# DecaYale/SYN3R

Hardware: AMD Instinct MI355X
Metric: llff_3view_train_loop_iters_per_sec (higher is better)
Workload: dtype f32 raster / f16 UNet (f32 accumulate); 1 GPU; LLFF fern-like 3-view block: 50 raster fwd+bwd iters (l1 loss) (200000 Gaussians, 1920x1080, SH3) + 1 SVD (step,pass): CFG UNet fwd [2,14,8,72,128] f16 + fused Euler step; frames=14, parallelism=scene-parallel x1

## Files before the change

### include/syn3r_hip.h

```cpp
#ifndef SYN3R_HIP_H
#define SYN3R_HIP_H

#include <stddef.h>
#include <stdint.h>

#ifdef __cplusplus
extern "C" {
#endif

#define SYN3R_OK 0
#define SYN3R_E_INVALID (-1)
#define SYN3R_E_WORKSPACE (-2)
#define SYN3R_E_HIP (-3)

#define SYN3R_F32 0
#define SYN3R_F16 1

const char* syn3r_last_error(void);
int syn3r_version(void);
const char* syn3r_arch(void);

int syn3r_trace_enable(int on);
void* syn3r_trace_session(void);
int syn3r_trace_attach(void* session);
// ... 114 lines not shown
                              const float* projmatrix, const float* campos, float tanfovx, float tanfovy, int H, int W,
                              const float* bg, const int* radii, void* geom, size_t geom_bytes,
                              const unsigned* point_list, void* image, size_t image_bytes, const float* dL_dcolor,
                              const float* dL_ddepth, const float* dL_dalpha, float* dL_dmeans3D, float* dL_dscales,
                              float* dL_drotations, float* dL_dopacities, float* dL_dshs, float* dL_dmeans2D,
                              float* dL_dconfidence, void* workspace, size_t workspace_bytes, int raw, int flags,
                              const float* filter3d, void* stream);
int syn3r_raster_backward_abs(int N, int sh_degree, int sh_coeffs, long long P, const float* means3D,
                              const float* scales, const float* rotations, const float* opacities, const float* shs,
                              const float* confidence, float scale_modifier, const float* viewmatrix,
                              const float* projmatrix, const float* campos, float tanfovx, float tanfovy, int H, int W,
                              const float* bg, const int* radii, void* geom, size_t geom_bytes,
                              const unsigned* point_list, void* image, size_t image_bytes, const float* dL_dcolor,
                              const float* dL_ddepth, const float* dL_dalpha, float* dL_dmeans3D, float* dL_dscales,
                              float* dL_drotations, float* dL_dopacities, float* dL_dshs, float* dL_dmeans2D,
                              float* dL_dconfidence, void* workspace, size_t workspace_bytes, int raw, int flags,
                              const float* filter3d, float* dL_dmeans2D_abs, void* stream);
size_t syn3r_raster_backward_cam_workspace_bytes(int N);
int syn3r_raster_backward_cam(int N, int sh_degree, int sh_coeffs, long long P, const float* means3D,
                              const float* scales, const float* rotations, const float* opacities, const float* shs,
                              const float* confidence, float scale_modifier, const float* viewmatrix,
                              const float* projmatrix, const float* campos, float tanfovx, float tanfovy, int H, int W,
                              const float* bg, const int* radii, void* geom, size_t geom_bytes,
                              const unsigned* point_list, void* image, size_t image_bytes, const float* dL_dcolor,
                              const float* dL_ddepth, const float* dL_dalpha, float* dL_dmeans3D, float* dL_dscales,
                              float* dL_drotations, float* dL_dopacities, float* dL_dshs, float* dL_dmeans2D,
                              float* dL_dconfidence, void* workspace, size_t workspace_bytes, int raw, int flags,
                              const float* filter3d, float* dL_dmeans2D_abs, float* dL_dcamera, int accumulate,
                              void* stream);

size_t syn3r_sort_pairs_workspace_bytes(long long n);
int syn3r_sort_pairs(unsigned long long* keys, unsigned* vals, unsigned long long* keys_tmp, unsigned* vals_tmp,
                     long long n, int nbits, void* workspace, size_t workspace_bytes, int* result_in_tmp,
                     void* stream);


int syn3r_gemm_f16(const void* A, long long lda, const void* W, void* out, long long ldc, const void* bias,
                   const void* rowvec, long long ldrv, int rows_per_vec, int rv_group_rows, const void* residual, long long ldr,
                   const void* aux, long long ldaux, float s_acc, float s_res, float s_aux, int M, int N, int K,
                   void* gn_partials, size_t gn_partials_bytes, int* gn_written, void* stream);

int syn3r_gemm_2src_supported(int M, int N, int K1, int K2, long long lda1, long long lda2);
int syn3r_gemm_2src_f16(const void* A1, long long lda1, int K1, const void* A2, long long lda2, int K2, const void* W,
                        void* out, long long ldc, const void* bias, int M, int N, void* gn_partials, size_t gn_partials_bytes,
                        int* gn_written, void* stream);

int syn3r_gemm_set_tile(int bm);

int syn3r_gemm_set_splitk_workspace(void* workspace, size_t bytes);

int syn3r_gemm_geglu_f16(const void* A, long long lda, const void* Wpacked, const void* bias_packed, void* out,
                         long long ldc, int M, int D, int K, void* stream);

size_t syn3r_feedforward_workspace_bytes(int M, int D);
int syn3r_feedforward_f16(const void* x, long long ldx, const void* w1_packed, const void* b1_packed, int D,
                          const void* w2, const void* b2, void* out, long long ldc, const void* residual,
                          long long ldr, const void* aux, long long ldaux, float s_acc, float s_res, float s_aux,
                          int M, int C_in, int C_out, void* workspace, size_t workspace_bytes, void* stream);

int syn3r_feedforward_p64_supported(int M, int D, int C_in);
int syn3r_feedforward_p64_f16(const void* x, long long ldx, const void* w1_packed64, const void* b1_packed64, int D,
                              const void* w2, const void* b2, void* out, long long ldc, const void* residual,
                              long long ldr, const void* aux, long long ldaux, float s_acc, float s_res, float s_aux,
                              int M, int C_in, int C_out, void* workspace, size_t workspace_bytes, void* stream);

int syn3r_feedforward_fused_f16(const void* x, long long ldx, const void* w1_chunked, const void* b1_chunked, int D,
                                const void* w2, const void* b2, void* out, long long ldc, const void* residual,
                                long long ldr, const void* aux, long long ldaux, float s_acc, float s_res, float s_aux,
                                int M, int C, void* stream);

int syn3r_feedforward_fused_ln_f16(const void* x, long long ldx, const void* ln_gamma, const void* ln_beta, float ln_eps,
                                   const void* w1_chunked, const void* b1_chunked, int D, const void* w2, const void* b2,
                                   void* out, long long ldc, const void* residual, long long ldr, const void* aux,
                                   long long ldaux, float s_acc, float s_res, float s_aux, int M, int C, void* stream);

int syn3r_feedforward_fused_addln_f16(const void* x, long long ldx, const void* addvec, int rows_per_vec, const void* ln_gamma,
                                      const void* ln_beta, float ln_eps, const void* w1_chunked, const void* b1_chunked, int D,
                                      const void* w2, const void* b2, void* out, long long ldc, const void* aux, long long ldaux,
                                      float s_acc, float s_res, float s_aux, int M, int C, void* stream);

int syn3r_layernorm_linear320_f16(const void* x, long long ldx, const void* ln_gamma, const void* ln_beta, float ln_eps,
                                  const void* W, void* out, long long ldc, int M, int N, int C, void* stream);

int syn3r_conv2d3x3_f16(const void* X, const void* W, void* out, long long ldc, const void* bias,
                        const void* rowvec, long long ldrv, int rows_per_vec, const void* residual, long long ldr,
                        float s_acc, float s_res, int NB, int Hi, int Wi, int Cin, int Cout, int stride, int upsample,
                        int pad_lo, void* gn_partials, size_t gn_partials_bytes, int* gn_written, void* stream);

int syn3r_pack_upsample4_f16(const void* w, void* w4, int Cout, int Cin);
int syn3r_conv2d3x3_up4_f16(const void* X, const void* w4, void* out, const void* bias, const void* residual, int NB, int Hi, int Wi,
                            int Cin, int Cout, void* gn_partials, size_t gn_partials_bytes, int* gn_written, void* stream);

int syn3r_tconv3_f16(const void* X, const void* W, void* out, long long ldc, const void* bias, const void* rowvec,
                     long long ldrv, int rows_per_vec, const void* residual, long long ldr, float s_acc, float s_res,
                     int B, int F, int HW, int Cin, int Cout, void* gn_partials, size_t gn_partials_bytes, int* gn_written,
                     void* stream);

int syn3r_attention_f16(const void* q, const void* k, const void* v, long long ld, void* out, long long ldo,
                        int nseq, int S, int heads, void* stream);

int syn3r_attention_temporal_f16(const void* q, const void* k, const void* v, long long ld, void* out,
                                 long long ldo, int B, int F, int HW, int heads, void* stream);

size_t syn3r_groupnorm_workspace_bytes(int samples, int rows);
int syn3r_groupnorm_f16(const void* x, void* y, int samples, int rows, int C, const void* gamma, const void* beta,
                        float eps, int silu, void* workspace, size_t workspace_bytes, void* stream);
int syn3r_groupnorm_2src_f16(const void* x1, int C1, const void* x2, int C2, void* y, int samples, int rows,
                             const void* gamma, const void* beta, float eps, int silu, void* workspace,
                             size_t workspace_bytes, void* stream);
size_t syn3r_gn_partials_bytes(int M, int N);
int syn3r_groupnorm_pre_f16(const void* x1, int C1, const void* part1, const void* x2, int C2, const void* part2, void* y,
                            int samples, int rows, const void* gamma, const void* beta, float eps, int silu,
                            void* workspace, size_t workspace_bytes, void* stream);

int syn3r_layernorm_f16(const void* x, void* y, void* xsum, const void* addvec, int rows_per_vec, long long M,
                        int C, const void* gamma, const void* beta, float eps, void* stream);

int syn3r_geglu_f16(const void* x, void* y, long long M, int D, void* stream);

int syn3r_softmax_rows_f16(const void* x, void* y, long long M, int N, long long ld, float scale, void* stream);

int syn3r_time_conv_out(const void* x, long long ldx, const float* w, const float* bias, float* out, int B, int F,
                        long long HW, void* stream);


size_t syn3r_l1_loss_workspace_bytes(long long n);
int syn3r_l1_loss(const float* image, const float* target, long long n, float weight, float* loss, void* ws,
                  size_t ws_bytes, void* stream);
int syn3r_l1_loss_backward(const float* image, const float* target, long long n, float weight,
                           const float* grad_loss, float* grad_image, void* stream);

int syn3r_image_mse(const float* image, const float* target, long long n, float* mse, void* ws, size_t ws_bytes,
                    void* stream);

size_t syn3r_photo_loss_workspace_bytes(int C, int H, int W);
int syn3r_photo_loss(const float* image, const float* target, int C, int H, int W, float lambda_dssim, float weight,
                     float* loss3, void* ws, size_t ws_bytes, void* stream);
int syn3r_photo_loss_backward(const float* image, const float* target, int C, int H, int W, float lambda_dssim,
                              float weight, const float* grad_loss, const void* ws, float* grad_image, void* stream);
int syn3r_photo_loss_step(const float* image, const float* target, int C, int H, int W, float lambda_dssim, float weight,
                          const float* grad_loss, float* loss3, float* grad_image, void* ws, size_t ws_bytes, void* stream);

size_t syn3r_photo_loss_map_workspace_bytes(int C, int H, int W);
int syn3r_photo_loss_map(const float* image, const float* target, const float* map, int C, int H, int W, float lambda_dssim,
                         float weight, float* loss4, void* ws, size_t ws_bytes, void* stream);
int syn3r_photo_loss_map_backward(const float* image, const float* target, const float* map, int C, int H, int W,
                                  float lambda_dssim, float weight, const float* grad_loss, const void* ws, float* grad_image,
                                  void* stream);
int syn3r_photo_loss_map_step(const float* image, const float* target, const float* map, int C, int H, int W, float lambda_dssim,
                              float weight, const float* grad_loss, float* loss4, float* grad_image, void* ws, size_t ws_bytes,
                              void* stream);
int syn3r_l1_loss_map(const float* image, const float* target, const float* map, long long n, long long plane, float weight,
                      float* loss, void* ws, size_t ws_bytes, void* stream);
int syn3r_l1_loss_map_backward(const float* image, const float* target, const float* map, long long n, long long plane,
                               float weight, const float* grad_loss, float* grad_image, void* stream);

#define SYN3R_DCORR_MIN 0
#define SYN3R_DCORR_A 1
#define SYN3R_DCORR_B 2
size_t syn3r_depth_corr_loss_workspace_bytes(long long n);
int syn3r_depth_corr_loss(const float* depth, const float* prior, long long n, float weight, float offset, int mode, float* parts,
                          void* ws, size_t ws_bytes, void* stream);
int syn3r_depth_corr_loss_backward(const float* depth, const float* prior, long long n, float weight, float offset, int mode,
                                   const float* grad_loss, const void* ws, size_t ws_bytes, float* grad_depth, void* stream);
int syn3r_depth_corr_loss_step(const float* depth, const float* prior, long long n, float weight, float offset, int mode,
                               const float* grad_loss, float* parts, float* grad_depth, void* ws, size_t ws_bytes, void* stream);
// ... 127 lines not shown
```

### syn3r_amd/_lib.py

```python
from __future__ import annotations

import ctypes as C
from pathlib import Path

import torch

_LIB_PATH = Path(__file__).resolve().parent / "lib" / "libsyn3r_hip.so"
_lib = None

c_f = C.c_float
c_i = C.c_int
c_p = C.c_void_p
c_sz = C.c_size_t
c_ll = C.c_longlong
c_d = C.c_double

F32, F16 = 0, 1
RASTER_ANTIALIAS = 1

FILTER3D_VARIANCE, FILTER3D_NEAR, FILTER3D_MARGIN = 0.2, 0.2, 0.15

_SCENE = [c_p, c_p, c_p, c_p, c_p, c_p, c_f, c_p, c_p, c_p, c_f, c_f, c_i, c_i]
_RASTER_PREPROCESS = [c_i, c_i, c_i] + _SCENE + [c_p, c_p, c_sz, C.POINTER(c_ll)]
_RASTER_BACKWARD = ([c_i, c_i, c_i, c_ll] + _SCENE + [c_p, c_p, c_p, c_sz, c_p, c_p, c_sz]
                    + [c_p] * 10 + [c_p, c_sz])
_STREAM, _EX, _F3D, _ABS = [c_p], [c_i, c_i, c_p], [c_i, c_i, c_p, c_p], [c_i, c_i, c_p, c_p, c_p]
_CAM = [c_i, c_i, c_p, c_p, c_p, c_i, c_p]
CAMERA_GRAD = 35

SIGNATURES = {
    "syn3r_last_error": (C.c_char_p, []),
    "syn3r_version": (c_i, []),
    "syn3r_arch": (C.c_char_p, []),
    "syn3r_trace_enable": (c_i, [c_i]),
    "syn3r_trace_filter": (c_i, [C.c_char_p]),
    "syn3r_trace_report": (c_i, [C.c_char_p, c_sz]),
    "syn3r_trace_session": (c_p, []),
    "syn3r_trace_attach": (c_i, [c_p]),
    "syn3r_inverse_warp_workspace_bytes": (c_sz, [c_i]),
    "syn3r_inverse_warp": (c_i, [c_p, c_p, c_p, c_p, c_p, c_p, c_p, c_f, c_i, c_i, c_i,
                                 c_p, c_p, c_p, c_p, c_p, c_p, c_p, c_p, c_p, c_p, c_p, c_p, c_sz, c_p]),
    "syn3r_reproj_error": (c_i, [c_p, c_p, c_p, c_p, c_p, c_p, c_p, c_i, c_i, c_p, c_p]),
    "syn3r_warp_post": (c_i, [c_p, c_p, c_p, c_i, c_i, c_i, c_i, c_i, c_p, c_p, c_p, c_p, c_p, c_p, c_p]),
    "syn3r_fuse_uncertainty": (c_i, [c_p, c_p, c_p, c_i, c_i, c_i, c_i, c_i, c_p, c_p, c_p, c_p]),
    "syn3r_forward_warp_workspace_bytes": (c_sz, [c_i, c_i]),
    "syn3r_forward_warp": (c_i, [c_p, c_p, c_p, c_p, c_p, c_p, c_i, c_i, c_p, c_p, c_p, c_p, c_sz, c_p]),
    "syn3r_step_workspace_bytes": (c_sz, [c_i, c_i, c_i, c_i]),
    "syn3r_step_interp": (c_i, [c_p, c_i, c_p, c_i, c_p, c_p, c_p, c_f, c_f, c_f, c_f, c_f, c_f, c_i,
                                c_p, c_p, c_p, c_i, c_i, c_i, c_i, c_p, c_sz, c_p]),
    "syn3r_step_replace": (c_i, [c_p, c_i, c_p, c_i, c_p, c_p, c_p, c_f, c_f, c_f, c_f,
                                 c_p, c_p, c_i, c_i, c_i, c_i, c_p, c_sz, c_p]),
    "syn3r_raster_geom_bytes": (c_sz, [c_i]),
    "syn3r_raster_image_bytes": (c_sz, [c_i, c_i]),
    "syn3r_raster_binning_bytes": (c_sz, [c_ll]),
    "syn3r_raster_preprocess": (c_i, _RASTER_PREPROCESS + _STREAM),
    "syn3r_raster_preprocess_raw": (c_i, _RASTER_PREPROCESS + _STREAM),
    "syn3r_raster_preprocess_ex": (c_i, _RASTER_PREPROCESS + _EX),
    "syn3r_raster_preprocess_f3d": (c_i, _RASTER_PREPROCESS + _F3D),
    "syn3r_raster_render": (c_i, [c_i, c_i, c_i, c_p, c_p, c_p, c_sz, c_p, c_sz, c_p, c_sz, c_ll, c_p, c_p, c_p,
                                  C.POINTER(c_p), c_p]),
    "syn3r_raster_backward_workspace_bytes": (c_sz, [c_i]),
    "syn3r_raster_backward": (c_i, _RASTER_BACKWARD + _STREAM),
    "syn3r_raster_backward_raw": (c_i, _RASTER_BACKWARD + _STREAM),
    "syn3r_raster_backward_ex": (c_i, _RASTER_BACKWARD + _EX),
    "syn3r_raster_backward_f3d": (c_i, _RASTER_BACKWARD + _F3D),
    "syn3r_raster_backward_abs": (c_i, _RASTER_BACKWARD + _ABS),
    "syn3r_raster_backward_cam_workspace_bytes": (c_sz, [c_i]),
    "syn3r_raster_backward_cam": (c_i, _RASTER_BACKWARD + _CAM),
    "syn3r_filter3d_workspace_bytes": (c_sz, [c_i]),
    "syn3r_filter3d_compute": (c_i, [c_p, c_i, c_p, c_i, c_f, c_f, c_f, c_p, c_p, c_sz, c_p]),
    "syn3r_sort_pairs_workspace_bytes": (c_sz, [c_ll]),
    "syn3r_sort_pairs": (c_i, [c_p, c_p, c_p, c_p, c_ll, c_i, c_p, c_sz, C.POINTER(c_i), c_p]),
    "syn3r_gaussian_activate": (c_i, [c_i, c_p, c_p, c_p, c_p, c_p, c_p, c_p]),
    "syn3r_gaussian_activate_backward": (c_i, [c_i, c_p, c_p, c_p, c_p, c_p, c_p, c_p, c_p, c_p, c_p, c_p]),
    "syn3r_densification_stats": (c_i, [c_i, c_p, c_p, c_p, c_p, c_p, c_p]),
    "syn3r_densification_stats_abs": (c_i, [c_i, c_p, c_p, c_p, c_p, c_p, c_p, c_p, c_p]),
    "syn3r_gemm_f16": (c_i, [c_p, c_ll, c_p, c_p, c_ll, c_p, c_p, c_ll, c_i, c_i, c_p, c_ll, c_p, c_ll, c_f, c_f, c_f,
                             c_i, c_i, c_i, c_p, c_sz, C.POINTER(c_i), c_p]),
    "syn3r_gemm_set_tile": (c_i, [c_i]),
    "syn3r_gemm_geglu_f16": (c_i, [c_p, c_ll, c_p, c_p, c_p, c_ll, c_i, c_i, c_i, c_p]),
    "syn3r_feedforward_workspace_bytes": (c_sz, [c_i, c_i]),
    "syn3r_feedforward_f16": (c_i, [c_p, c_ll, c_p, c_p, c_i, c_p, c_p, c_p, c_ll, c_p, c_ll, c_p, c_ll, c_f, c_f, c_f,
                                    c_i, c_i, c_i, c_p, c_sz, c_p]),
    "syn3r_feedforward_p64_f16": (c_i, [c_p, c_ll, c_p, c_p, c_i, c_p, c_p, c_p, c_ll, c_p, c_ll, c_p, c_ll, c_f, c_f, c_f,
                                    c_i, c_i, c_i, c_p, c_sz, c_p]),
    "syn3r_feedforward_p64_supported": (c_i, [c_i, c_i, c_i]),
    "syn3r_feedforward_fused_f16": (c_i, [c_p, c_ll, c_p, c_p, c_i, c_p, c_p, c_p, c_ll, c_p, c_ll, c_p, c_ll, c_f, c_f, c_f,
                                          c_i, c_i, c_p]),
    "syn3r_feedforward_fused_ln_f16": (c_i, [c_p, c_ll, c_p, c_p, c_f, c_p, c_p, c_i, c_p, c_p, c_p, c_ll, c_p, c_ll, c_p, c_ll,
                                             c_f, c_f, c_f, c_i, c_i, c_p]),
    "syn3r_feedforward_fused_addln_f16": (c_i, [c_p, c_ll, c_p, c_i, c_p, c_p, c_f, c_p, c_p, c_i, c_p, c_p, c_p, c_ll, c_p, c_ll,
                                                c_f, c_f, c_f, c_i, c_i, c_p]),
    "syn3r_layernorm_linear320_f16": (c_i, [c_p, c_ll, c_p, c_p, c_f, c_p, c_p, c_ll, c_i, c_i, c_i, c_p]),
    "syn3r_conv2d3x3_f16": (c_i, [c_p, c_p, c_p, c_ll, c_p, c_p, c_ll, c_i, c_p, c_ll, c_f, c_f,
                                  c_i, c_i, c_i, c_i, c_i, c_i, c_i, c_i, c_p, c_sz, C.POINTER(c_i), c_p]),
    "syn3r_pack_upsample4_f16": (c_i, [c_p, c_p, c_i, c_i]),
    "syn3r_conv2d3x3_up4_f16": (c_i, [c_p, c_p, c_p, c_p, c_p, c_i, c_i, c_i, c_i, c_i, c_p, c_sz, C.POINTER(c_i), c_p]),
    "syn3r_tconv3_f16": (c_i, [c_p, c_p, c_p, c_ll, c_p, c_p, c_ll, c_i, c_p, c_ll, c_f, c_f,
                               c_i, c_i, c_i, c_i, c_i, c_p, c_sz, C.POINTER(c_i), c_p]),
    "syn3r_attention_f16": (c_i, [c_p, c_p, c_p, c_ll, c_p, c_ll, c_i, c_i, c_i, c_p]),
    "syn3r_attention_temporal_f16": (c_i, [c_p, c_p, c_p, c_ll, c_p, c_ll, c_i, c_i, c_i, c_i, c_p]),
    "syn3r_groupnorm_workspace_bytes": (c_sz, [c_i, c_i]),
    "syn3r_groupnorm_f16": (c_i, [c_p, c_p, c_i, c_i, c_i, c_p, c_p, c_f, c_i, c_p, c_sz, c_p]),
    "syn3r_groupnorm_2src_f16": (c_i, [c_p, c_i, c_p, c_i, c_p, c_i, c_i, c_p, c_p, c_f, c_i, c_p, c_sz, c_p]),
    "syn3r_groupnorm_pre_f16": (c_i, [c_p, c_i, c_p, c_p, c_i, c_p, c_p, c_i, c_i, c_p, c_p, c_f, c_i, c_p, c_sz, c_p]),
    "syn3r_gn_partials_bytes": (c_sz, [c_i, c_i]),
    "syn3r_gemm_2src_supported": (c_i, [c_i, c_i, c_i, c_i, c_ll, c_ll]),
    "syn3r_gemm_2src_f16": (c_i, [c_p, c_ll, c_i, c_p, c_ll, c_i, c_p, c_p, c_ll, c_p, c_i, c_i, c_p, c_sz, C.POINTER(c_i), c_p]),
    "syn3r_layernorm_f16": (c_i, [c_p, c_p, c_p, c_p, c_i, c_ll, c_i, c_p, c_p, c_f, c_p]),
    "syn3r_geglu_f16": (c_i, [c_p, c_p, c_ll, c_i, c_p]),
    "syn3r_softmax_rows_f16": (c_i, [c_p, c_p, c_ll, c_i, c_ll, c_f, c_p]),
    "syn3r_time_conv_out": (c_i, [c_p, c_ll, c_p, c_p, c_p, c_i, c_i, c_ll, c_p]),
    "syn3r_l1_loss_workspace_bytes": (c_sz, [c_ll]),
    "syn3r_l1_loss": (c_i, [c_p, c_p, c_ll, c_f, c_p, c_p, c_sz, c_p]),
    "syn3r_l1_loss_backward": (c_i, [c_p, c_p, c_ll, c_f, c_p, c_p, c_p]),
    "syn3r_image_mse": (c_i, [c_p, c_p, c_ll, c_p, c_p, c_sz, c_p]),
    "syn3r_photo_loss_workspace_bytes": (c_sz, [c_i, c_i, c_i]),
    "syn3r_photo_loss": (c_i, [c_p, c_p, c_i, c_i, c_i, c_f, c_f, c_p, c_p, c_sz, c_p]),
    "syn3r_photo_loss_backward": (c_i, [c_p, c_p, c_i, c_i, c_i, c_f, c_f, c_p, c_p, c_p, c_p]),
    "syn3r_photo_loss_step": (c_i, [c_p, c_p, c_i, c_i, c_i, c_f, c_f, c_p, c_p, c_p, c_p, c_sz, c_p]),
    "syn3r_photo_loss_map_workspace_bytes": (c_sz, [c_i, c_i, c_i]),
    "syn3r_photo_loss_map": (c_i, [c_p, c_p, c_p, c_i, c_i, c_i, c_f, c_f, c_p, c_p, c_sz, c_p]),
    "syn3r_photo_loss_map_backward": (c_i, [c_p, c_p, c_p, c_i, c_i, c_i, c_f, c_f, c_p, c_p, c_p, c_p]),
    "syn3r_photo_loss_map_step": (c_i, [c_p, c_p, c_p, c_i, c_i, c_i, c_f, c_f, c_p, c_p, c_p, c_p, c_sz, c_p]),
    "syn3r_l1_loss_map": (c_i, [c_p, c_p, c_p, c_ll, c_ll, c_f, c_p, c_p, c_sz, c_p]),
    "syn3r_l1_loss_map_backward": (c_i, [c_p, c_p, c_p, c_ll, c_ll, c_f, c_p, c_p, c_p]),
    "syn3r_depth_corr_loss_workspace_bytes": (c_sz, [c_ll]),
    "syn3r_depth_corr_loss": (c_i, [c_p, c_p, c_ll, c_f, c_f, c_i, c_p, c_p, c_sz, c_p]),
    "syn3r_depth_corr_loss_backward": (c_i, [c_p, c_p, c_ll, c_f, c_f, c_i, c_p, c_p, c_sz, c_p, c_p]),
    "syn3r_depth_corr_loss_step": (c_i, [c_p, c_p, c_ll, c_f, c_f, c_i, c_p, c_p, c_p, c_p, c_sz, c_p]),
    "syn3r_depth_corr_local_workspace_bytes": (c_sz, [c_i, c_i, c_i, c_i, c_i]),
    "syn3r_depth_corr_local_loss": (c_i, [c_p, c_p, c_i, c_i, c_i, c_i, c_i, c_f, c_f, c_i, c_p, c_p, c_sz, c_p]),
    "syn3r_depth_corr_local_loss_backward": (c_i, [c_p, c_p, c_i, c_i, c_i, c_i, c_i, c_f, c_f, c_i, c_p, c_p, c_sz, c_p, c_i, c_p]),
    "syn3r_depth_corr_local_loss_step": (c_i, [c_p, c_p, c_i, c_i, c_i, c_i, c_i, c_f, c_f, c_i, c_p, c_p, c_p, c_i, c_p, c_sz, c_p]),
    "syn3r_exposure_apply": (c_i, [c_p, c_p, c_i, c_i, c_p, c_p]),
    "syn3r_depth_edge_weights": (c_i, [c_p, c_i, c_i, c_f, c_p, c_p]),
    "syn3r_depth_smooth_workspace_bytes": (c_sz, [c_i, c_i]),
    "syn3r_depth_smooth_loss": (c_i, [c_p, c_p, c_i, c_i, c_f, c_p, c_p, c_sz, c_p]),
    "syn3r_depth_smooth_loss_backward": (c_i, [c_p, c_p, c_i, c_i, c_f, c_p, c_p, c_sz, c_p, c_i, c_p]),
    "syn3r_depth_smooth_loss_step": (c_i, [c_p, c_p, c_i, c_i, c_f, c_p, c_p, c_p, c_i, c_p, c_sz, c_p]),
    "syn3r_photo_reproj_workspace_bytes": (c_sz, [c_i, c_i, c_i]),
    "syn3r_photo_reproj_loss": (c_i, [c_p, c_p, c_p, c_p, c_p, c_p, c_i, c_i, c_i, c_f, c_f, c_p, c_p, c_sz, c_p]),
    "syn3r_photo_reproj_loss_backward": (c_i, [c_p, c_p, c_i, c_i, c_i, c_f, c_f, c_p, c_p, c_sz, c_p, c_i, c_p, c_i, c_p]),
    "syn3r_photo_reproj_loss_step": (c_i, [c_p, c_p, c_p, c_p, c_p, c_p, c_i, c_i, c_i, c_f, c_f, c_p, c_p, c_p, c_i, c_p, c_i, c_p, c_sz,
                                           c_p]),
    "syn3r_exposure_backward_workspace_bytes": (c_sz, [c_i, c_i]),
    "syn3r_exposure_backward": (c_i, [c_p, c_p, c_p, c_i, c_i, c_p, c_p, c_i, c_p, c_sz, c_p]),
    "syn3r_mcmc_noise": (c_i, [c_p, c_p, c_p, c_p, c_i, c_f, c_ll, c_i, c_p]),
    "syn3r_mcmc_reg_step_workspace_bytes": (c_sz, [c_i]),
    "syn3r_mcmc_reg_step": (c_i, [c_p, c_p, c_i, c_f, c_f, c_p, c_p, c_p, c_p, c_sz, c_p]),
    "syn3r_mcmc_weights": (c_i, [c_p, c_i, c_f, c_p, c_p]),
    "syn3r_mcmc_sample_workspace_bytes": (c_sz, [c_i]),
    "syn3r_mcmc_sample": (c_i, [c_p, c_i, c_i, c_ll, c_i, c_p, c_p, c_p, c_sz, c_p]),
    "syn3r_mcmc_relocate": (c_i, [c_i, c_p, c_p, c_p, c_p, c_i, c_p, c_p, c_p, c_p, c_f, c_p]),
    "syn3r_adam_step": (c_i, [c_p, c_p, c_p, c_p, c_ll, c_f, c_f, c_f, c_f, c_i, c_p]),
    "syn3r_adam_step_multi": (c_i, [c_i, c_p, c_p, c_p, c_p, c_p, c_p, c_f, c_f, c_p, c_p, c_p]),
    "syn3r_adam_step_multi_rows": (c_i, [c_i, c_p, c_p, c_p, c_p, c_p, c_p, c_p, c_p, c_p, c_f, c_f, c_p, c_p, c_p]),
    "syn3r_knn3_workspace_bytes": (c_sz, [c_i]),
    "syn3r_knn3_mean_dist2": (c_i, [c_p, c_i, c_p, c_p, c_sz, c_p]),
    "syn3r_knn3_graph_workspace_bytes": (c_sz, [c_i]),
    "syn3r_knn3_graph": (c_i, [c_p, c_i, c_p, c_p, c_p, c_sz, c_p]),
    "syn3r_gaussian_unpool_workspace_bytes": (c_sz, [c_i]),
    "syn3r_gaussian_unpool_count": (c_i, [c_p, c_p, c_i, c_f, c_f, c_p, c_p, c_sz, c_p]),
    "syn3r_gaussian_unpool_emit": (c_i, [c_p, c_p, c_p, c_p, c_p, c_i, c_i, c_i, c_p, c_p, c_p, c_p, c_p, c_p, c_sz, c_p]),
    "syn3r_conv2d3x3_act_f16": (c_i, [c_p, c_p, c_p, c_p, c_i, c_p, c_i, c_i, c_i, c_i, c_i, c_p]),
    "syn3r_lpips_image_f16": (c_i, [c_p, c_i, c_i, c_p, c_p]),
    "syn3r_lpips_image_bwd": (c_i, [c_p, c_i, c_i, c_f, c_p, c_p]),
    "syn3r_maxpool2_f16": (c_i, [c_p, c_i, c_i, c_i, c_p, c_p]),
    "syn3r_maxpool2_bwd_f16": (c_i, [c_p, c_p, c_i, c_i, c_i, c_p, c_p]),
    "syn3r_lpips_layer_workspace_bytes": (c_sz, [c_ll, c_i]),
    "syn3r_lpips_layer_f16": (c_i, [c_p, c_p, c_p, c_ll, c_i, c_i, c_p, c_p, c_sz, c_p]),
    "syn3r_lpips_layer_bwd_f16": (c_i, [c_p, c_p, c_p, c_ll, c_i, c_f, c_i, c_p, c_p]),
    "syn3r_conv2d3x3_split_f16": (c_i, [c_p, c_p, c_p, c_ll, c_p, c_i, c_i, c_p, c_ll, c_i, c_i, c_i, c_i, c_i, c_p]),
    "syn3r_lpips_image_split_f16": (c_i, [c_p, c_i, c_i, c_p, c_p]),
    "syn3r_maxpool2_split_f16": (c_i, [c_p, c_i, c_i, c_i, c_p, c_p]),
    "syn3r_maxpool2_bwd_split_f16": (c_i, [c_p, c_p, c_i, c_i, c_i, c_p, c_p]),
# ... 144 lines not shown
```

### syn3r_amd/csrc/attn.hip

```cpp
#include "common.h"
#include <type_traits>

using namespace syn3r;

namespace {

typedef _Float16 half8 __attribute__((ext_vector_type(8)));
typedef _Float16 half4 __attribute__((ext_vector_type(4)));
typedef float float16v __attribute__((ext_vector_type(16)));
typedef float float2v __attribute__((ext_vector_type(2)));
typedef __fp16 fp16x4 __attribute__((__vector_size__(4 * sizeof(__fp16))));

__device__ __forceinline__ int v_off(int key, int d) { return key * 64 + ((((d >> 3) ^ (((key >> 1) & 1) << 2)) << 3) | (d & 7)); }
__device__ __forceinline__ int k_off(int key, int chunk) { return key * 64 + ((chunk ^ ((key >> 1) & 7)) << 3); }

__device__ __forceinline__ half8 v_frag_tr(const __half* vs, int r0, int d0, int lane) {
    const int i = lane & 15, q = i >> 2, pc = i & 3;
    const int c = d0 + ((lane >> 4) & 1) * 16 + 4 * pc;
    typedef __attribute__((address_space(3))) fp16x4 lds4;
    fp16x4 a = __builtin_amdgcn_ds_read_tr16_b64_v4f16((lds4*)(vs + v_off(r0 + q, c)));
    fp16x4 b = __builtin_amdgcn_ds_read_tr16_b64_v4f16((lds4*)(vs + v_off(r0 + 8 + q, c)));
    half8 r;
#pragma unroll
    for (int e = 0; e < 4; ++e) { r[e] = (_Float16)a[e]; r[4 + e] = (_Float16)b[e]; }
    return r;
}

constexpr float kNegBig = -1.0e30f;
constexpr float kLog2e = 1.4426950408889634f;
constexpr float kLazy = 8.0f;

__device__ __forceinline__ half8 pack8(const float16v& p, int s) {
    half8 r;
#pragma unroll
    for (int j = 0; j < 8; ++j) r[j] = (_Float16)p[8 * s + j];
    return r;
}

struct AttnParams {
    const __half* q; const __half* k; const __half* v;
    long long ld;
    __half* o; long long ldo;
    int S;
    int nseq;
    int heads;
    int F, HW;
};

constexpr int BQ = 128, BKV = 64, ATHREADS = 256;

typedef float float4v __attribute__((ext_vector_type(4)));
typedef __attribute__((address_space(3))) void lds_void_t;
typedef __attribute__((address_space(1))) const void gbl_void_t;

#ifndef ATTN_WAVES
#define ATTN_WAVES 3
#endif
__device__ __forceinline__ float max3(float a, float b, float c) {
    float d;
    asm("v_max3_f32 %0, %1, %2, %3" : "=v"(d) : "v"(a), "v"(b), "v"(c));
    return d;
}
__device__ __forceinline__ int v16_off(int key, int d) { return key * 64 + ((((d >> 4) ^ ((key >> 1) & 3)) << 4) | (d & 15)); }

__device__ __forceinline__ half8 v16_frag_tr(const __half* vs, int r0, int d0, int lane) {
    const int i = lane & 15, q = i >> 2, pc = i & 3;
    const int c = d0 + 4 * pc;
    typedef __attribute__((address_space(3))) fp16x4 lds4;
    fp16x4 a = __builtin_amdgcn_ds_read_tr16_b64_v4f16((lds4*)(vs + v16_off(r0 + q, c)));
    fp16x4 b = __builtin_amdgcn_ds_read_tr16_b64_v4f16((lds4*)(vs + v16_off(r0 + 16 + q, c)));
    half8 r;
#pragma unroll
    for (int e = 0; e < 4; ++e) { r[e] = (_Float16)a[e]; r[4 + e] = (_Float16)b[e]; }
    return r;
}

__global__ void __launch_bounds__(ATHREADS, ATTN_WAVES) k_attn_spatial(AttnParams p) {
    __shared__ __attribute__((aligned(1024))) __half Ks[2][BKV * 64];
    __shared__ __attribute__((aligned(1024))) __half Vs[2][BKV * 64];
    const int tid = threadIdx.x, lane = tid & 63, wv = __builtin_amdgcn_readfirstlane(tid >> 6);
    const int l16 = lane & 15, g4 = lane >> 4;
    const int qblocks = (p.S + BQ - 1) / BQ;
    int bid = (int)xcd_remap(blockIdx.x, gridDim.x);
    const int qb = bid % qblocks; bid /= qblocks;
    const int hd = bid % p.heads;
    const int seq = bid / p.heads;
    const long long row0 = (long long)seq * p.S;
    const int q0 = qb * BQ + wv * 32;
    const __half* qp = p.q + hd * 64;
    const __half* kp = p.k + hd * 64 + row0 * p.ld;
    const __half* vp = p.v + hd * 64 + row0 * p.ld;

    half8 qf[2][2];
#pragma unroll
    for (int qg = 0; qg < 2; ++qg) {
        int qi = q0 + qg * 16 + l16;
        if (qi > p.S - 1) qi = p.S - 1;
        const __half* src = qp + (row0 + qi) * p.ld;
#pragma unroll
        for (int ks = 0; ks < 2; ++ks) {
            half8 t = *(const half8*)(src + ks * 32 + 8 * g4);
#pragma unroll
            for (int j = 0; j < 8; ++j) t[j] = (_Float16)((float)t[j] * (0.125f * kLog2e));
            qf[qg][ks] = t;
        }
    }

    unsigned ok[2], ov[2];
    const int s_key = wv * 16 + (lane >> 3), s_c = lane & 7;
    const unsigned ldb = (unsigned)p.ld * 2u;
#pragma unroll
    for (int i = 0; i < 2; ++i) {
        const int key = s_key + 8 * i;
        ok[i] = (unsigned)key * ldb + (unsigned)((s_c ^ ((key >> 1) & 7)) << 4);
        ov[i] = (unsigned)key * ldb + (unsigned)((s_c ^ (((key >> 1) & 3) << 1)) << 4);
    }
    auto dma_tile = [&](int kv0, int buf) {
        long long tile_off = (long long)kv0 * p.ld * 2;
        asm volatile("" : "+s"(tile_off));
        const char* kb = (const char*)kp + tile_off;
// ... 72 lines not shown
        }
        float mq[2];
#pragma unroll
        for (int qg = 0; qg < 2; ++qg) {
            float a = max3(st[0][qg][0], st[0][qg][1], st[0][qg][2]), b = max3(st[1][qg][0], st[1][qg][1], st[1][qg][2]);
            float c = max3(st[2][qg][0], st[2][qg][1], st[2][qg][2]), d = max3(st[3][qg][0], st[3][qg][1], st[3][qg][2]);
            a = max3(a, st[0][qg][3], st[1][qg][3]);
            c = max3(c, st[2][qg][3], st[3][qg][3]);
            mq[qg] = max3(max3(a, b, c), d, d);
        }
        const bool first = t == 0;
        if (first || __ballot(fmaxf(mq[0], mq[1]) > kLazy) != 0ull) {
#pragma unroll
            for (int qg = 0; qg < 2; ++qg) {
                float mx = mq[qg];
                {
                    auto sw = __builtin_amdgcn_permlane32_swap(__float_as_int(mx), __float_as_int(mx), false, false);
                    mx = fmaxf(__int_as_float(sw[0]), __int_as_float(sw[1]));
                    auto sx = __builtin_amdgcn_permlane16_swap(__float_as_int(mx), __float_as_int(mx), false, false);
                    mx = fmaxf(__int_as_float(sx[0]), __int_as_float(sx[1]));
                }
                const float delta = first ? mx : fmaxf(mx, 0.f);
                if (!first) {
                    const float alpha = __builtin_amdgcn_exp2f(-delta);
#pragma unroll
                    for (int dt = 0; dt < 4; ++dt)
#pragma unroll
                        for (int r = 0; r < 4; ++r) ot[dt][qg][r] *= alpha;
#pragma unroll
                    for (int r = 0; r < 4; ++r) lsum[qg][r] *= alpha;
                }
#pragma unroll
                for (int kg = 0; kg < 4; ++kg)
#pragma unroll
                    for (int r = 0; r < 4; ++r) st[kg][qg][r] -= delta;
#pragma unroll
                for (int r = 0; r < 4; ++r) negm[qg][r] -= delta;
            }
        }
#pragma unroll
        for (int kg = 0; kg < 4; ++kg)
#pragma unroll
            for (int qg = 0; qg < 2; ++qg)
#pragma unroll
                for (int r = 0; r < 4; ++r) st[kg][qg][r] = __builtin_amdgcn_exp2f(st[kg][qg][r]);
#pragma unroll
        for (int G = 0; G < 2; ++G)
#pragma unroll
            for (int qg = 0; qg < 2; ++qg) {
                half8 pf;
#pragma unroll
                for (int j = 0; j < 4; ++j) { pf[j] = (_Float16)st[2 * G][qg][j]; pf[4 + j] = (_Float16)st[2 * G + 1][qg][j]; }
                lsum[qg] = __builtin_amdgcn_mfma_f32_16x16x32_f16(ones8, pf, lsum[qg], 0, 0, 0);
#pragma unroll
                for (int dt = 0; dt < 4; ++dt) ot[dt][qg] = __builtin_amdgcn_mfma_f32_16x16x32_f16(vf[G][dt], pf, ot[dt][qg], 0, 0, 0);
            }
        __builtin_amdgcn_s_waitcnt(0x0F70);
        __syncthreads();
    };
    dma_tile(0, 0);
    __builtin_amdgcn_s_waitcnt(0x0F70);
    __syncthreads();
    for (int t = 0; t < ntiles; t += 2) {
        tile(t, std::integral_constant<int, 0>{});
        if (t + 1 < ntiles) tile(t + 1, std::integral_constant<int, 1>{});
    }
#pragma unroll
    for (int qg = 0; qg < 2; ++qg) {
        const float inv = 1.0f / lsum[qg][0];
        const int qi = q0 + qg * 16 + l16;
        if (qi < p.S) {
            __half* dst = p.o + (row0 + qi) * p.ldo + hd * 64;
#pragma unroll
            for (int dt = 0; dt < 4; ++dt) {
                half4 o4;
#pragma unroll
                for (int e = 0; e < 4; ++e) o4[e] = (_Float16)(ot[dt][qg][e] * inv);
                *(half4*)(dst + dt * 16 + 4 * g4) = o4;
            }
        }
    }
}

__global__ void __launch_bounds__(ATHREADS, 2) k_attn_temporal(AttnParams p, long long nitems) {
    __shared__ __attribute__((aligned(16))) __half Vsm[4][32 * 64];
    const int tid = threadIdx.x, lane = tid & 63, wv = tid >> 6;
    const int lq = lane & 31, h = lane >> 5;
    long long item = (long long)blockIdx.x * 4 + wv;
    const bool live = item < nitems;
    if (!live) item = nitems - 1;
    const int hd = (int)(item % p.heads);
    long long bp = item / p.heads;
    const int pix = (int)(bp % p.HW);
    const int b = (int)(bp / p.HW);
    const int F = p.F;
    auto row_of = [&](int f) { return ((long long)b * F + f) * p.HW + pix; };

    const int fq = lq < F ? lq : F - 1;
    const __half* qsrc = p.q + row_of(fq) * p.ld + hd * 64;
    const __half* ksrc = p.k + row_of(fq) * p.ld + hd * 64;
    half8 qf[4], kf[4];
#pragma unroll
    for (int ks = 0; ks < 4; ++ks) {
        half8 t = *(const half8*)(qsrc + ks * 16 + 8 * h);
#pragma unroll
        for (int j = 0; j < 8; ++j) t[j] = t[j] * (_Float16)0.125f;
        qf[ks] = t;
        kf[ks] = *(const half8*)(ksrc + ks * 16 + 8 * h);
    }
    __half* vs = Vsm[wv];
#pragma unroll
    for (int i = 0; i < 4; ++i) {
        int q = lane + 64 * i;
        int key = q >> 3, ch = q & 7;
        uint4 rv = make_uint4(0, 0, 0, 0);
        if (key < F) rv = *(const uint4*)(p.v + row_of(key) * p.ld + hd * 64 + ch * 8);
        *(uint4*)(vs + v_off(key, ch * 8)) = rv;
    }
    float16v st;
#pragma unroll
    for (int r = 0; r < 16; ++r) st[r] = 0.f;
#pragma unroll
    for (int ks = 0; ks < 4; ++ks) st = __builtin_amdgcn_mfma_f32_32x32x16_f16(kf[ks], qf[ks], st, 0, 0, 0);
    float mx = kNegBig;
#pragma unroll
    for (int r = 0; r < 16; ++r) {
        int key = (r & 3) + 8 * (r >> 2) + 4 * h;
        if (key >= F) st[r] = kNegBig;
        mx = fmaxf(mx, st[r]);
    }
    mx = fmaxf(mx, __shfl_xor(mx, 32, 64));
    float ls = 0.f;
#pragma unroll
    for (int r = 0; r < 16; ++r) {
        float e = __expf(st[r] - mx);
        st[r] = e;
        ls += e;
    }
    ls += __shfl_xor(ls, 32, 64);
    __syncthreads();
    float16v ot[2];
#pragma unroll
    for (int r = 0; r < 16; ++r) { ot[0][r] = 0.f; ot[1][r] = 0.f; }
#pragma unroll
    for (int s = 0; s < 2; ++s) {
        half8 pf = pack8(st, s);
#pragma unroll
        for (int dt = 0; dt < 2; ++dt) {
            half8 vf = v_frag_tr(vs, s * 16 + 4 * h, dt * 32, lane);
            ot[dt] = __builtin_amdgcn_mfma_f32_32x32x16_f16(vf, pf, ot[dt], 0, 0, 0);
        }
    }
    if (live && lq < F) {
        const float inv = 1.0f / ls;
        __half* dst = p.o + row_of(lq) * p.ldo + hd * 64;
#pragma unroll
        for (int dt = 0; dt < 2; ++dt)
#pragma unroll
            for (int g = 0; g < 4; ++g) {
                half4 o4;
#pragma unroll
                for (int e = 0; e < 4; ++e) o4[e] = (_Float16)(ot[dt][4 * g + e] * inv);
                *(half4*)(dst + dt * 32 + 8 * g + 4 * h) = o4;
            }
    }
}

}

extern "C" int syn3r_attention_f16(const void* q, const void* k, const void* v, long long ld, void* out, long long ldo,
                                   int nseq, int S, int heads, void* stream) {
    SYN3R_REQUIRE(q && k && v && out, "attention: null tensor");
    SYN3R_REQUIRE(SYN3R_DIM_OK(nseq) && SYN3R_DIM_OK(S) && heads > 0 && heads <= 4096, "attention: bad sizes nseq=%d S=%d heads=%d", nseq, S, heads);
    SYN3R_REQUIRE(ld % 8 == 0 && ldo % 8 == 0 && ld >= 64 * heads && ldo >= 64 * heads, "attention: bad strides");
    SYN3R_REQUIRE(ld < (1ll << 24), "attention: row stride %lld too large (the K / V tile offsets 64 * ld * 2 are 32-bit)", ld);
    SYN3R_REQUIRE(((uintptr_t)q | (uintptr_t)k | (uintptr_t)v | (uintptr_t)out) % 16 == 0, "attention: misaligned tensor");
    AttnParams p{};
    p.q = (const __half*)q; p.k = (const __half*)k; p.v = (const __half*)v; p.ld = ld;
    p.o = (__half*)out; p.ldo = ldo; p.S = S; p.nseq = nseq; p.heads = heads;
    long long blocks = (long long)nseq * heads * ((S + BQ - 1) / BQ);
    SYN3R_REQUIRE(blocks < (1ll << 31), "attention: grid too large");
    SYN3R_LAUNCH(k_attn_spatial, dim3((unsigned)blocks), dim3(ATHREADS), 0, (hipStream_t)stream, p);
    SYN3R_LAUNCH_CHECK("attention launch");
    return SYN3R_OK;
}

extern "C" int syn3r_attention_temporal_f16(const void* q, const void* k, const void* v, long long ld, void* out,
                                            long long ldo, int B, int F, int HW, int heads, void* stream) {
    SYN3R_REQUIRE(q && k && v && out, "attention_temporal: null tensor");
    SYN3R_REQUIRE(SYN3R_DIM_OK(B) && SYN3R_DIM_OK(HW) && heads > 0 && heads <= 4096 && F >= 1 && F <= 32, "attention_temporal: bad sizes B=%d F=%d HW=%d heads=%d (F <= 32)",
                  B, F, HW, heads);
    SYN3R_REQUIRE(ld % 8 == 0 && ldo % 8 == 0 && ld >= 64 * heads && ldo >= 64 * heads, "attention_temporal: bad strides");
    SYN3R_REQUIRE(((uintptr_t)q | (uintptr_t)k | (uintptr_t)v | (uintptr_t)out) % 16 == 0, "attention_temporal: misaligned tensor");
    AttnParams p{};
    p.q = (const __half*)q; p.k = (const __half*)k; p.v = (const __half*)v; p.ld = ld;
    p.o = (__half*)out; p.ldo = ldo; p.S = F; p.heads = heads; p.F = F; p.HW = HW;
    long long nitems = (long long)B * HW * heads;
    long long blocks = (nitems + 3) / 4;
    SYN3R_REQUIRE(blocks < (1ll << 31), "attention_temporal: grid too large");
    SYN3R_LAUNCH(k_attn_temporal, dim3((unsigned)blocks), dim3(ATHREADS), 0, (hipStream_t)stream, p, nitems);
    SYN3R_LAUNCH_CHECK("attention_temporal launch");
    return SYN3R_OK;
}
```

### syn3r_amd/csrc/gemm.hip

```cpp
#include "common.h"
#include <cstdlib>
#include <algorithm>
#include <atomic>
#include <type_traits>

using namespace syn3r;

namespace {

#include "gemm_common.h"
#include "gemm_dma160.h"
#include "gemm_dma.h"
#include "gemm_wide.h"
#include "gemm_z.h"
#include "gemm_dmap.h"
#include "gemm_dmapd.h"
#include "gemm_g256.h"
#include "gemm_ffn.h"

int persistent_blocks() {
    static std::atomic<int> cus_of[64];
    static const int forced = tune_env("SYN3R_PERSISTENT_BLOCKS", 0);
    if (forced > 0) return forced < 8 ? 8 : forced;
    int dev = 0;
    if (hipGetDevice(&dev) != hipSuccess || dev < 0 || dev >= 64) dev = 0;
    int n = cus_of[dev].load(std::memory_order_relaxed);
    if (n == 0) {
        int v = 0;
        n = (hipDeviceGetAttribute(&v, hipDeviceAttributeMultiprocessorCount, dev) == hipSuccess && v > 0) ? v : 256;
        if (n < 8) n = 8;
        cus_of[dev].store(n, std::memory_order_relaxed);
    }
    return n;
}

size_t gn_partials_bytes(long long M, long long N) { return (size_t)(M / 32) * 2 * (size_t)(N / 10) * sizeof(float); }
int gn_request(GemmParams& p, void* buf, size_t bytes, const char* who) {
    SYN3R_REQUIRE((buf == nullptr) == (bytes == 0), "%s: gn_partials pointer and size must both be given or both be zero", who);
    SYN3R_REQUIRE(((uintptr_t)buf % 16) == 0, "%s: the gn_partials buffer must be 16-byte aligned", who);
    if (!buf || p.M % 32 != 0 || p.N % 80 != 0 || p.geglu_D > 0 || p.out_tiled || bytes < gn_partials_bytes(p.M, p.N)) return SYN3R_OK;
    p.gn_part = (float*)buf; p.gn_units = p.N / 10;
    return SYN3R_OK;
}

template <void (*KERNEL)(GemmParams)>
int launch_tiles(const char* family, size_t lds, long long grid, int block, hipStream_t stream, const GemmParams& q, int* gn_written,
                 const char* base, int b0 = 0, int b1 = 0) {
    static DevOnce once;
    if (int rc = set_max_lds(once, (const void*)KERNEL, (int)lds, family)) return rc;
    char name[96];
    if (trace_on()) {
        const int n = snprintf(name, sizeof(name), base, b0, b1);
        if (trace_detail()) snprintf(name + n, sizeof(name) - n, "[M%d,N%d,K%d,e%d]", q.M, q.N, q.K, q.geglu_D > 0 ? 2 : (q.residual != nullptr));
    }
    SYN3R_LAUNCH_NAMED(name, KERNEL, dim3((unsigned)grid), dim3(block), lds, stream, q);
    hipError_t e = hipGetLastError();
    if (e != hipSuccess) { set_error("%s launch: %s", family, hipGetErrorString(e)); return SYN3R_E_HIP; }
    if (gn_written) *gn_written = q.gn_part != nullptr;
    return SYN3R_OK;
}

long long wide_tiles(const GemmParams& p) { return (long long)((p.M + WBM - 1) / WBM) * ((p.N + WBN - 1) / WBN); }
bool wide_fills(const GemmParams& p) {
    const long long tiles = wide_tiles(p), rounds = (tiles + 255) / 256;
    return tiles * 10 >= rounds * 256 * 8;
}

int band_width(const GemmParams& p) {
    static const int band_env = tune_env("SYN3R_Z_BAND", 0);
    if (band_env > 0) return band_env;
    return ((p.N + WBN - 1) / WBN > 4 && p.K <= 640) ? 3 : 4;
}

int launch_widep(const GemmParams& p, hipStream_t stream, int* gn_written) {
    constexpr size_t lds = (size_t)2 * W_STAGE + 16384;
    static_assert(8 * WM * EPI_LD * sizeof(__half) <= lds - W_STAGE, "epilogue staging must fit behind ring slot 0");
    GemmParams q = p;
    q.band = band_width(p);
    return launch_tiles<k_gemm_widep>("gemm_widep", lds, std::min<long long>(wide_tiles(p), persistent_blocks()), 512, stream, q, gn_written, "k_gemm_widep");
}

bool g256_admits(const GemmParams& p) {
    return p.geglu_D > 0 && p.bias != nullptr && p.out_tiled && !p.a_tiled && !p.A2 && !p.rowvec && !p.residual && !p.aux && p.s_acc == 1.0f && p.M % 128 == 0 && p.M >= 256 &&
           p.geglu_D % 128 == 0 && p.N == 2 * p.geglu_D && p.K >= 2 * BK && p.lda % 8 == 0 && (long long)p.M * p.lda < (1ll << 31) &&
           (long long)p.N * p.K < (1ll << 31);
}
int launch_g256(const GemmParams& p, hipStream_t stream) {
    const int tiles = ((p.M + 255) / 256) * (p.N / 256);
    GemmParams q = p;
    static const int band_env = tune_env("SYN3R_G256_BAND", 0);
    q.band = band_env > 0 ? band_env : 4;
    return launch_tiles<k_gemm_g256>("gemm_g256", G_LDS, std::min(tiles, persistent_blocks()), 512, stream, q, nullptr, "k_gemm_g256");
}

template <int MODE = MODE_DENSE>
int launch_z(const GemmParams& p, hipStream_t stream, int* gn_written) {
    const long long blocks = std::min<long long>(wide_tiles(p), persistent_blocks());
    GemmParams q = p;
    q.band = band_width(p);
    if constexpr (MODE == MODE_CONV2D) q.a_bytes = (unsigned)((long long)(p.M / (p.Ho * p.Wo)) * p.Hi * p.Wi * p.Cin * 2);
    if constexpr (MODE == MODE_TCONV) q.a_bytes = (unsigned)((long long)p.M * p.Cin * 2);
// ... 347 lines not shown
    p.bias = (const __half*)b1_packed64; p.s_acc = 1.0f; p.M = M; p.N = 2 * D; p.K = C_in; p.geglu_D = D; p.out_tiled = 1;
    p.out_nt = need >= ((size_t)256 << 20);
    int rc = check_common(p, "feedforward_p64_f16(net.0)");
    if (rc) return rc;
    SYN3R_REQUIRE(g256_admits(p), "feedforward_p64_f16: shape not admitted by the 256 x 256 kernel");
    rc = launch_g256(p, (hipStream_t)stream);
    if (rc) return rc;
    return ffn_net2("feedforward_p64_f16(net.2)", workspace, D, w2, b2, out, ldc, residual, ldr, aux, ldaux, s_acc, s_res, s_aux, M, C_out, (hipStream_t)stream);
}

namespace {
int feedforward_fused(const void* x, long long ldx, const void* ln_gamma, const void* ln_beta, float ln_eps, const void* w1_chunked,
                      const void* b1_chunked, int D, const void* w2, const void* b2, void* out, long long ldc, const void* residual,
                      long long ldr, const void* aux, long long ldaux, float s_acc, float s_res, float s_aux, int M, int C, void* stream,
                      const void* addvec = nullptr, int rows_per_vec = 0);
}
extern "C" int syn3r_feedforward_fused_f16(const void* x, long long ldx, const void* w1_chunked, const void* b1_chunked,
                                           int D, const void* w2, const void* b2, void* out, long long ldc,
                                           const void* residual, long long ldr, const void* aux, long long ldaux,
                                           float s_acc, float s_res, float s_aux, int M, int C, void* stream) {
    return feedforward_fused(x, ldx, nullptr, nullptr, 0.f, w1_chunked, b1_chunked, D, w2, b2, out, ldc, residual, ldr, aux, ldaux,
                             s_acc, s_res, s_aux, M, C, stream);
}
extern "C" int syn3r_feedforward_fused_ln_f16(const void* x, long long ldx, const void* ln_gamma, const void* ln_beta, float ln_eps,
                                              const void* w1_chunked, const void* b1_chunked, int D, const void* w2, const void* b2,
                                              void* out, long long ldc, const void* residual, long long ldr, const void* aux,
                                              long long ldaux, float s_acc, float s_res, float s_aux, int M, int C, void* stream) {
    SYN3R_REQUIRE(ln_gamma && ln_beta, "feedforward_fused_ln_f16: null LayerNorm parameters");
    SYN3R_REQUIRE(((uintptr_t)ln_gamma | (uintptr_t)ln_beta) % 16 == 0, "feedforward_fused_ln_f16: LayerNorm parameters must be 16-byte aligned");
    SYN3R_REQUIRE(ln_eps > 0.f, "feedforward_fused_ln_f16: eps must be positive");
    return feedforward_fused(x, ldx, ln_gamma, ln_beta, ln_eps, w1_chunked, b1_chunked, D, w2, b2, out, ldc, residual, ldr, aux, ldaux,
                             s_acc, s_res, s_aux, M, C, stream);
}
extern "C" int syn3r_feedforward_fused_addln_f16(const void* x, long long ldx, const void* addvec, int rows_per_vec, const void* ln_gamma,
                                                 const void* ln_beta, float ln_eps, const void* w1_chunked, const void* b1_chunked, int D,
                                                 const void* w2, const void* b2, void* out, long long ldc, const void* aux, long long ldaux,
                                                 float s_acc, float s_res, float s_aux, int M, int C, void* stream) {
    SYN3R_REQUIRE(ln_gamma && ln_beta && addvec, "feedforward_fused_addln_f16: null LayerNorm parameters / add vector");
    SYN3R_REQUIRE(((uintptr_t)ln_gamma | (uintptr_t)ln_beta | (uintptr_t)addvec) % 16 == 0, "feedforward_fused_addln_f16: LayerNorm parameters and the add vector must be 16-byte aligned");
    SYN3R_REQUIRE(ln_eps > 0.f, "feedforward_fused_addln_f16: eps must be positive");
    SYN3R_REQUIRE(rows_per_vec > 0, "feedforward_fused_addln_f16: rows_per_vec=%d must be positive", rows_per_vec);
    return feedforward_fused(x, ldx, ln_gamma, ln_beta, ln_eps, w1_chunked, b1_chunked, D, w2, b2, out, ldc, x, ldx, aux, ldaux,
                             s_acc, s_res, s_aux, M, C, stream, addvec, rows_per_vec);
}
namespace {
int feedforward_fused(const void* x, long long ldx, const void* ln_gamma, const void* ln_beta, float ln_eps, const void* w1_chunked,
                      const void* b1_chunked, int D, const void* w2, const void* b2, void* out, long long ldc, const void* residual,
                      long long ldr, const void* aux, long long ldaux, float s_acc, float s_res, float s_aux, int M, int C, void* stream,
                      const void* addvec, int rows_per_vec) {
    SYN3R_REQUIRE(x && w1_chunked && b1_chunked && w2 && out, "feedforward_fused_f16: null operand");
    SYN3R_REQUIRE(C == F_C, "feedforward_fused_f16: the fused kernel is built for C = %d channels (got %d): use syn3r_feedforward_f16", F_C, C);
    SYN3R_REQUIRE(M > 0 && D >= F_HC && D % F_HC == 0, "feedforward_fused_f16: bad sizes M=%d D=%d (D must be a multiple of %d)", M, D, F_HC);
    FfnParams q{};
    GemmParams& p = q.e;
    p.A = (const __half*)x; p.lda = ldx; p.W = (const __half*)w2; p.out = (__half*)out; p.ldc = ldc;
    p.bias = (const __half*)b2; p.residual = (const __half*)residual; p.ldr = ldr; p.aux = (const __half*)aux; p.ldaux = ldaux;
    p.s_acc = s_acc; p.s_res = s_res; p.s_aux = s_aux; p.M = M; p.N = F_C; p.K = D;
    q.w1 = (const __half*)w1_chunked; q.b1 = (const __half*)b1_chunked; q.D = D;
    q.ln_g = (const __half*)ln_gamma; q.ln_b = (const __half*)ln_beta; q.ln_eps = ln_eps;
    q.ln_add = (const __half*)addvec; q.ln_add_rpv = rows_per_vec; p.res_add = (const __half*)addvec; p.res_add_rpv = rows_per_vec;
    int rc = check_common(p, "feedforward_fused_f16");
    if (rc) return rc;
    SYN3R_REQUIRE(ldx % 8 == 0 && ldx >= C, "feedforward_fused_f16: ldx=%lld must be >= C and a multiple of 8", ldx);
    SYN3R_REQUIRE(((uintptr_t)w1_chunked | (uintptr_t)b1_chunked) % 16 == 0, "feedforward_fused_f16: weights must be 16-byte aligned");
    return launch_ffn320(q, (hipStream_t)stream);
}
}

extern "C" int syn3r_layernorm_linear320_f16(const void* x, long long ldx, const void* ln_gamma, const void* ln_beta, float ln_eps,
                                             const void* W, void* out, long long ldc, int M, int N, int C, void* stream) {
    SYN3R_REQUIRE(x && ln_gamma && ln_beta && W && out, "layernorm_linear320_f16: null operand");
    SYN3R_REQUIRE(C == F_C, "layernorm_linear320_f16: the kernel is built for C = %d channels (got %d): use syn3r_layernorm_f16 + syn3r_gemm_f16", F_C, C);
    SYN3R_REQUIRE(SYN3R_DIM_OK(M) && SYN3R_DIM_OK(N) && N % F_C == 0, "layernorm_linear320_f16: bad sizes M=%d N=%d (N must be a multiple of %d)", M, N, F_C);
    SYN3R_REQUIRE(ldx % 8 == 0 && ldx >= C && ldc % 8 == 0 && ldc >= N, "layernorm_linear320_f16: bad strides ldx=%lld ldc=%lld", ldx, ldc);
    SYN3R_REQUIRE(((uintptr_t)x | (uintptr_t)ln_gamma | (uintptr_t)ln_beta | (uintptr_t)W | (uintptr_t)out) % 16 == 0, "layernorm_linear320_f16: operands must be 16-byte aligned");
    SYN3R_REQUIRE(ln_eps > 0.f, "layernorm_linear320_f16: eps must be positive");
    SYN3R_REQUIRE((long long)M * ldx < (1ll << 40) && (long long)M * ldc < (1ll << 40), "layernorm_linear320_f16: operand too large");
    LnLinParams p{};
    p.x = (const __half*)x; p.ldx = ldx; p.W = (const __half*)W; p.out = (__half*)out; p.ldc = ldc; p.M = M; p.N = N; p.C = C;
    p.ln_g = (const __half*)ln_gamma; p.ln_b = (const __half*)ln_beta; p.ln_eps = ln_eps;
    return launch_lnlin320(p, (hipStream_t)stream);
}

extern "C" int syn3r_conv2d3x3_f16(const void* X, const void* W, void* out, long long ldc, const void* bias,
                                   const void* rowvec, long long ldrv, int rows_per_vec, const void* residual,
                                   long long ldr, float s_acc, float s_res, int NB, int Hi, int Wi, int Cin, int Cout,
                                   int stride, int upsample, int pad_lo, void* gn_partials, size_t gn_partials_bytes, int* gn_written,
                                   void* stream) {
    if (gn_written) *gn_written = 0;
    SYN3R_REQUIRE(NB > 0 && Hi > 0 && Wi > 0 && Cin > 0 && Cout > 0, "conv2d3x3: bad sizes");
    SYN3R_REQUIRE(pad_lo == 0 || pad_lo == 1, "conv2d3x3: pad_lo must be 0 or 1");
    SYN3R_REQUIRE(stride == 1 || stride == 2, "conv2d3x3: stride must be 1 or 2");
    SYN3R_REQUIRE(!(upsample && stride != 1), "conv2d3x3: upsample requires stride 1");
    SYN3R_REQUIRE(Cin % BK == 0, "conv2d3x3: Cin=%d must be a multiple of %d (pad the input channels)", Cin, BK);
    GemmParams p{};
    p.A = (const __half*)X; p.W = (const __half*)W; p.out = (__half*)out; p.ldc = ldc; p.bias = (const __half*)bias;
    p.rowvec = (const __half*)rowvec; p.ldrv = ldrv; p.rows_per_vec = rows_per_vec;
    p.residual = (const __half*)residual; p.ldr = ldr; p.s_acc = s_acc; p.s_res = s_res; p.s_aux = 0.f;
    p.Hi = Hi; p.Wi = Wi; p.Cin = Cin; p.stride = stride; p.ups = upsample ? 1 : 0; p.pad = pad_lo;
    int Hg = upsample ? 2 * Hi : Hi, Wg = upsample ? 2 * Wi : Wi;
    p.Ho = (Hg + pad_lo + 1 - 3) / stride + 1;
    p.Wo = (Wg + pad_lo + 1 - 3) / stride + 1;
    SYN3R_REQUIRE(p.Ho > 0 && p.Wo > 0, "conv2d3x3: input too small");
    long long M = (long long)NB * p.Ho * p.Wo;
    SYN3R_REQUIRE(M < (1ll << 31), "conv2d3x3: too many output pixels");
    p.M = (int)M; p.N = Cout; p.K = 9 * Cin;
    int rc = gn_request(p, gn_partials, gn_partials_bytes, "conv2d3x3");
    if (rc) return rc;
    rc = check_common(p, "conv2d3x3");
    if (rc) return rc;
    return launch_dma<MODE_CONV2D>(p, (hipStream_t)stream, gn_written);
}

extern "C" int syn3r_conv2d3x3_up4_f16(const void* X, const void* W4, void* out, const void* bias, const void* residual, int NB, int Hi,
                                       int Wi, int Cin, int Cout, void* gn_partials, size_t gn_partials_bytes, int* gn_written,
                                       void* stream) {
    if (gn_written) *gn_written = 0;
    SYN3R_REQUIRE(X && W4 && out, "conv2d3x3_up4: null operand");
    SYN3R_REQUIRE(!residual, "conv2d3x3_up4: the phase form takes no residual (use syn3r_conv2d3x3_f16 with upsample = 1)");
    SYN3R_REQUIRE(SYN3R_DIM_OK(NB) && SYN3R_SIDE_OK(Hi) && SYN3R_SIDE_OK(Wi) && SYN3R_DIM_OK(Cin) && SYN3R_DIM_OK(Cout), "conv2d3x3_up4: bad sizes");
    SYN3R_REQUIRE(Cin % BK == 0, "conv2d3x3_up4: Cin=%d must be a multiple of %d (a k-tile is %d channels of one tap)", Cin, BK, BK);
    SYN3R_REQUIRE(Cout % 8 == 0, "conv2d3x3_up4: Cout=%d must be a multiple of 8", Cout);
    const long long M4 = (long long)NB * Hi * Wi;
    SYN3R_REQUIRE(M4 < (1ll << 24), "conv2d3x3_up4: %lld input pixels (the phase form takes fewer than 2^24)", M4);
    SYN3R_REQUIRE(M4 * Cin * 2 < (1ll << 32) - (1 << 20) && (long long)Cout * 4 * Cin < (1ll << 29), "conv2d3x3_up4: operand too large");
    SYN3R_REQUIRE(((uintptr_t)X | (uintptr_t)W4 | (uintptr_t)out | (uintptr_t)bias) % 16 == 0, "conv2d3x3_up4: operands must be 16-byte aligned");
    SYN3R_REQUIRE((gn_partials == nullptr) == (gn_partials_bytes == 0), "conv2d3x3_up4: gn_partials pointer and size must both be given or both be zero");
    SYN3R_REQUIRE(((uintptr_t)gn_partials % 16) == 0, "conv2d3x3_up4: the gn_partials buffer must be 16-byte aligned");
    GemmParams p{};
    p.A = (const __half*)X; p.W = (const __half*)W4; p.out = (__half*)out; p.ldc = Cout; p.bias = (const __half*)bias;
    p.s_acc = 1.0f; p.s_res = 0.f; p.s_aux = 0.f;
    p.Hi = Hi; p.Wi = Wi; p.Cin = Cin; p.stride = 1; p.ups = 0; p.pad = 1; p.Ho = Hi; p.Wo = Wi;
    p.M = (int)M4; p.N = Cout; p.K = 4 * Cin;
    if (gn_partials && ((long long)Hi * Wi) % 32 == 0 && Cout % 80 == 0 && gn_partials_bytes >= ::gn_partials_bytes(4 * M4, Cout)) {
        p.gn_part = (float*)gn_partials; p.gn_units = Cout / 10; p.up4_bpi = Hi * Wi / 32;
    }
    return launch_z_up4(p, (hipStream_t)stream, gn_written);
}

namespace {
int conv3x3_act_params(const char* who, const void* X, const void* W, void* out, long long ldc, const void* bias, int relu, const void* relu_mask,
                       long long ld_mask, int NB, int Hi, int Wi, int Cin, int Cout, GemmParams& p) {
    SYN3R_REQUIRE(NB > 0 && Hi > 0 && Wi > 0 && Cin > 0 && Cout > 0, "%s: bad sizes", who);
    SYN3R_REQUIRE(Cin % BK == 0 && Cout % 8 == 0, "%s: Cin=%d must be a multiple of %d, Cout=%d of 8", who, Cin, BK, Cout);
    p.A = (const __half*)X; p.W = (const __half*)W; p.out = (__half*)out; p.ldc = ldc; p.bias = (const __half*)bias;
    p.s_acc = 1.0f; p.s_res = 0.f; p.s_aux = 0.f;
    p.relu = relu ? 1 : 0; p.relu_mask = (const __half*)relu_mask; p.ld_mask = (int)ld_mask;
    p.Hi = Hi; p.Wi = Wi; p.Cin = Cin; p.stride = 1; p.ups = 0; p.pad = 1; p.Ho = Hi; p.Wo = Wi;
    long long M = (long long)NB * Hi * Wi;
    SYN3R_REQUIRE(M < (1ll << 31), "%s: too many output pixels", who);
    p.M = (int)M; p.N = Cout; p.K = 9 * Cin;
    return check_common(p, who);
}
}

extern "C" int syn3r_conv2d3x3_act_f16(const void* X, const void* W, void* out, const void* bias, int relu, const void* relu_mask,
                                       int NB, int Hi, int Wi, int Cin, int Cout, void* stream) {
    GemmParams p{};
    if (int rc = conv3x3_act_params("conv2d3x3_act", X, W, out, Cout, bias, relu, relu_mask, 0, NB, Hi, Wi, Cin, Cout, p)) return rc;
    SYN3R_REQUIRE(((uintptr_t)relu_mask % 16) == 0, "conv2d3x3_act: mask must be 16-byte aligned");
    return launch_dma<MODE_CONV2D>(p, (hipStream_t)stream);
}

extern "C" int syn3r_conv2d3x3_split_f16(const void* X, const void* W, void* out, long long ld_out, const void* bias, int relu, int split_out,
                                         const void* relu_mask, long long ld_mask, int NB, int Hi, int Wi, int Cin, int Cout, void* stream) {
    SYN3R_REQUIRE(ld_out >= (split_out ? 2ll : 1ll) * Cout, "conv2d3x3_split: ld_out=%lld is short of %d columns", ld_out, (split_out ? 2 : 1) * Cout);
// ... 42 lines not shown
```

### syn3r_amd/csrc/unet.hip

```cpp
#include "common.h"
#include "unet_ckpt.h"
#include <exception>
#include <map>
#include <memory>
#include <algorithm>
#include <unordered_set>
#include <mutex>

using namespace syn3r;

namespace {

__global__ void k_timestep_embedding(const float* __restrict__ t_dev, double t_host, float t_step, int n, int dim, __half* __restrict__ out) {
    const int half = dim / 2;
    const int i = blockIdx.x * blockDim.x + threadIdx.x;
    if (i >= n * half) return;
    const int r = i / half, c = i - r * half;
    const float t = t_dev ? t_dev[r] : (float)t_host + t_step * (float)r;
    const float e = expf((-9.210340371976184f * (float)c) * (1.0f / (float)half));
    const float a = t * e;
    out[(size_t)r * dim + c] = __float2half(cosf(a));
    out[(size_t)r * dim + half + c] = __float2half(sinf(a));
}
__global__ void k_silu(const __half* __restrict__ x, __half* __restrict__ y, long long n) {
    const long long i = (long long)blockIdx.x * blockDim.x + threadIdx.x;
    if (i >= n) return;
    const float v = __half2float(x[i]);
    y[i] = __float2half(v / (1.0f + expf(-v)));
}
__global__ void k_add(const __half* __restrict__ a, const __half* __restrict__ b, __half* __restrict__ y, long long n) {
    const long long i = (long long)blockIdx.x * blockDim.x + threadIdx.x;
    if (i < n) y[i] = __float2half(__half2float(a[i]) + __half2float(b[i]));
}
__global__ void k_nchw_to_nhwc(const __half* __restrict__ x, __half* __restrict__ y, int N, int C, int hw, int CP) {
    const long long i = (long long)blockIdx.x * blockDim.x + threadIdx.x;
    if (i >= (long long)N * hw * CP) return;
    const int c = (int)(i % CP);
    const long long pix = i / CP;
    const int n = (int)(pix / hw), p = (int)(pix - (long long)n * hw);
    y[i] = c < C ? x[((long long)n * C + c) * hw + p] : __float2half(0.f);
}
__global__ void k_nhwc_to_nchw(const __half* __restrict__ x, __half* __restrict__ y, int N, int C, int hw, int CP) {
    const long long i = (long long)blockIdx.x * blockDim.x + threadIdx.x;
    if (i >= (long long)N * C * hw) return;
    const int p = (int)(i % hw);
    const long long nc = i / hw;
    const int n = (int)(nc / C), c = (int)(nc - (long long)n * C);
    y[i] = x[((long long)n * hw + p) * CP + c];
}
__global__ void k_repeat_rows(const __half* __restrict__ x, __half* __restrict__ y, int rows_in, long long rows_out, int C) {
    const long long i = (long long)blockIdx.x * blockDim.x + threadIdx.x;
    if (i >= rows_out * C) return;
    const long long r = i / C;
    y[i] = x[(r % rows_in) * C + (i - r * C)];
}
__global__ void k_cat_cols(const __half* __restrict__ a, int C1, const __half* __restrict__ b, int C2, __half* __restrict__ y, long long M) {
    const int C = C1 + C2;
    const long long i = (long long)blockIdx.x * blockDim.x + threadIdx.x;
    if (i >= M * C) return;
    const long long r = i / C;
    const int c = (int)(i - r * C);
    y[i] = c < C1 ? a[r * C1 + c] : b[r * C2 + (c - C1)];
}

struct Wt { __half* p = nullptr; long long rows = 0, cols = 0; };

}

struct syn3r_unet : Checkpoint {
    int device = 0;
    char* blob = nullptr; size_t blob_bytes = 0;
    std::unordered_map<std::string, Wt> w;
    struct PosEmb { __half* p = nullptr; hipEvent_t ready = nullptr; hipStream_t stream = nullptr; };
    std::map<std::string, PosEmb> pos_cache;
    bool ff_ln = true, ln_qkv = true;
};

namespace {

std::mutex g_unet_mu;
std::unordered_set<const syn3r_unet*>& unet_registry() { static auto* s = new std::unordered_set<const syn3r_unet*>; return *s; }
bool unet_live(const syn3r_unet* m) {
    std::lock_guard<std::mutex> lk(g_unet_mu);
    return m && unet_registry().count(m);
}

int unet_create_impl(const char* weights_dir, const char* variant, syn3r_unet** out) {
    std::unique_ptr<syn3r_unet> m(new syn3r_unet);
    int rc = load_checkpoint(weights_dir, variant, *m);
    if (rc) return rc;
    rc = check_hip(hipGetDevice(&m->device), "hipGetDevice");
    if (rc) return rc;
    size_t total = 0;
    for (auto& hp : m->packs) total += (hp.d.size() * 2 + 255) / 256 * 256;
    rc = check_hip(hipMalloc((void**)&m->blob, total ? total : 256), "hipMalloc(unet weights)");
    if (rc) return rc;
    m->blob_bytes = total;
    size_t off = 0;
    for (auto& hp : m->packs) {
        rc = check_hip(hipMemcpy(m->blob + off, hp.d.data(), hp.d.size() * 2, hipMemcpyHostToDevice), "hipMemcpy(unet weights)");
        if (rc) { (void)hipFree(m->blob); return rc; }
        m->w[hp.name] = Wt{(__half*)(m->blob + off), hp.rows, hp.cols};
        off += (hp.d.size() * 2 + 255) / 256 * 256;
    }
    std::vector<HostPack>().swap(m->packs);
    m->ff_ln = tune_env("SYN3R_FF_LN", 1) != 0;
    m->ln_qkv = tune_env("SYN3R_LN_QKV", 1) != 0;
    *out = m.release();
    {
        std::lock_guard<std::mutex> lk(g_unet_mu);
        unet_registry().insert(*out);
    }
    return SYN3R_OK;
}

}

extern "C" int syn3r_unet_create(const char* weights_dir, const char* variant, syn3r_unet** out) {
    SYN3R_REQUIRE(weights_dir && out, "unet_create: null argument");
    *out = nullptr;
    try {
        return unet_create_impl(weights_dir, variant, out);
    } catch (const std::exception& e) {
        set_error("unet_create: %s", e.what());
    } catch (...) {
        set_error("unet_create: unexpected exception");
    }
    *out = nullptr;
    return SYN3R_E_INVALID;
}

extern "C" int syn3r_unet_destroy(syn3r_unet* m) {
    if (!m) return SYN3R_OK;
    {
        std::lock_guard<std::mutex> lk(g_unet_mu);
        if (!unet_registry().erase(m)) { set_error("unet_destroy: not a live handle"); return SYN3R_E_INVALID; }
    }
    for (auto& kv : m->pos_cache) {
        if (kv.second.ready) (void)hipEventDestroy(kv.second.ready);
        (void)hipFree(kv.second.p);
    }
    if (m->blob) (void)hipFree(m->blob);
    delete m;
    return SYN3R_OK;
}

namespace {

struct Arena {
    char* base = nullptr; size_t cap = 0, peak = 0;
    std::map<size_t, size_t> free_;
    std::unordered_map<size_t, size_t> live;
    void reset(char* b, size_t c) { base = b; cap = c; peak = 0; free_.clear(); live.clear(); free_[0] = c; }
    void* alloc(size_t n) {
        n = (n + 255) / 256 * 256;
        if (!n) n = 256;
        for (auto it = free_.begin(); it != free_.end(); ++it) {
            if (it->second >= n) {
                const size_t off = it->first, rest = it->second - n;
                free_.erase(it);
                if (rest) free_[off + n] = rest;
                live[off] = n;
                peak = std::max(peak, off + n);
                return base + off;
            }
        }
        return nullptr;
    }
    void release(void* p) {
        if (!p) return;
        size_t off = (size_t)((char*)p - base);
        auto it = live.find(off);
        if (it == live.end()) return;
        size_t n = it->second;
        live.erase(it);
        auto nx = free_.lower_bound(off);
        if (nx != free_.end() && off + n == nx->first) { n += nx->second; nx = free_.erase(nx); }
        if (nx != free_.begin()) {
            auto pv = std::prev(nx);
            if (pv->first + pv->second == off) { pv->second += n; return; }
        }
        free_[off] = n;
    }
};

struct T { __half* p = nullptr; long long rows = 0; int cols = 0; float* gnp = nullptr; int gn_ok = 0; };

struct Epi {
    const __half* rowvec = nullptr; long long ldrv = 0; int rows_per_vec = 0, rv_group = 0;
    const T* residual = nullptr; const T* aux = nullptr;
// ... 249 lines not shown
        if (own_skip) drop(skip);
        T g1 = groupnorm(xs, t + ".norm1", B, 1e-5f, true);
        Epi e3; slice(t + ".time_emb_proj", e3);
        T c1 = tconv3(g1, t + ".conv1.weight", t + ".conv1.bias", HW, e3);
        drop(g1);
        T g2 = groupnorm(c1, t + ".norm2", B, 1e-5f, true);
        drop(c1);
        double a, om;
        blend(pre, a, om);
        Epi e4; e4.residual = &xs; e4.s_acc = (float)om; e4.s_res = (float)(a + om);
        T out = tconv3(g2, t + ".conv2.weight", t + ".conv2.bias", HW, e4);
        drop(g2);
        drop(xs);
        return out;
    }

    const __half* pos_embedding(const std::string& pre, int ch) {
        const std::string key = pre + "|" + std::to_string(F) + "|" + std::to_string(B);
        auto it = m.pos_cache.find(key);
        if (it != m.pos_cache.end() && !dry) {
            if (it->second.stream != stream && it->second.ready) chk(check_hip(hipStreamWaitEvent(stream, it->second.ready, 0), "hipStreamWaitEvent(position embedding)"));
            return it->second.p;
        }
        T pos = make(F, ch);
        launch1d(k_timestep_embedding, F * (ch / 2), (const float*)nullptr, 0.0, 1.0f, F, ch, pos.p);
        T e2 = embed_mlp(pre + ".time_pos_embed", pos);
        __half* keep = nullptr;
        if (go()) {
            chk(check_hip(hipMalloc((void**)&keep, (size_t)B * F * ch * 2), "hipMalloc(position embedding)"));
            if (ok()) {
                launch1d(k_repeat_rows, (long long)B * F * ch, e2.p, keep, F, (long long)B * F, ch);
                syn3r_unet::PosEmb pe;
                pe.p = keep; pe.stream = stream;
                if (hipEventCreateWithFlags(&pe.ready, hipEventDisableTiming) == hipSuccess) {
                    if (hipEventRecord(pe.ready, stream) != hipSuccess) { (void)hipEventDestroy(pe.ready); pe.ready = nullptr; }
                } else pe.ready = nullptr;
                m.pos_cache[key] = pe;
            } else if (keep) { (void)hipFree(keep); keep = nullptr; }
        }
        drop(e2);
        return keep;
    }

    T transformer(const std::string& pre, const T& x, int ch, int heads) {
        const int HW = h * w;
        T gn = groupnorm(x, pre + ".norm", B * F, 1e-6f, false);
        T hs = linear(gn, pre + ".proj_in.weight", pre + ".proj_in.bias");
        drop(gn);
        const __half* emb = pos_embedding(pre, ch);
        const std::string b = pre + ".transformer_blocks.0", t = pre + ".temporal_transformer_blocks.0";
        {
            T qkv = norm_qkv(b, hs);
            T a1 = attention(qkv, B * F, HW, heads);
            drop(qkv);
            const T& cv = cross_vec(b + ".attn2");
            Epi e; e.residual = &hs; e.rowvec = dry ? nullptr : cv.p; e.ldrv = cv.cols; e.rows_per_vec = (shared_ctx ? B : 1) * F * HW;
            T o = linear(a1, b + ".attn1.to_out.0.weight", b + ".attn1.to_out.0.bias", e);
            drop(a1);
            drop(hs);
            hs = o;
            Epi ef; ef.residual = &hs;
            T f2 = ff(b + ".ff", hs, b + ".norm3", ef);
            drop(hs);
            hs = f2;
        }
        T tt;
        if (m.ff_ln && m.w.count(t + ".ff_in.net.0.proj.geglu_cw")) {
            tt = make(hs.rows, hs.cols);
            const Wt* w0 = W(t + ".ff_in.net.0.proj.weight");
            if (go())
                chk(syn3r_feedforward_fused_addln_f16(hs.p, hs.cols, emb, HW, Wp(t + ".norm_in.weight"), Wp(t + ".norm_in.bias"), 1e-5f,
                                                      Wp(t + ".ff_in.net.0.proj.geglu_cw"), Wp(t + ".ff_in.net.0.proj.geglu_cb"), w0 ? (int)(w0->rows / 2) : 0,
                                                      Wp(t + ".ff_in.net.2.weight"), Wp(t + ".ff_in.net.2.bias"), tt.p, tt.cols, nullptr, 0, 1.f, 1.f, 0.f,
                                                      (int)hs.rows, hs.cols, stream));
        } else {
            T hmix;
            T nin = layernorm(hs, t + ".norm_in", emb, HW, &hmix);
            Epi e0; e0.residual = &hmix;
            tt = ff(t + ".ff_in", nin, "", e0);
            drop(nin);
            drop(hmix);
        }
        {
            T qkv = norm_qkv(t, tt);
            T a1 = attention_temporal(qkv, HW, heads);
            drop(qkv);
            int rpv, grp;
            if (shared_ctx) { rpv = B * F * HW; grp = 0; }
            else if (G == 1) { rpv = F * HW; grp = 0; }
            else {
                if (HW % G && !rc) { set_error("unet_forward: the temporal cross-attention context interleave needs h*w divisible by the group size %d", G); rc = SYN3R_E_INVALID; }
                rpv = -G; grp = G != B ? G * F * HW : 0;
            }
            const T& cv = cross_vec(t + ".attn2");
            Epi e; e.residual = &tt; e.rowvec = dry ? nullptr : cv.p; e.ldrv = cv.cols; e.rows_per_vec = rpv; e.rv_group = grp;
            T o = linear(a1, t + ".attn1.to_out.0.weight", t + ".attn1.to_out.0.bias", e);
            drop(a1);
            drop(tt);
            tt = o;
        }
        double a, om;
        blend(pre, a, om);
        Epi em; em.residual = &tt; em.aux = &hs; em.s_acc = (float)om; em.s_res = (float)om; em.s_aux = (float)a;
        T mix = ff(t + ".ff", tt, t + ".norm3", em);
        drop(tt);
        drop(hs);
        Epi eo; eo.residual = &x;
        T out = linear(mix, pre + ".proj_out.weight", pre + ".proj_out.bias", eo, true);
        drop(mix);
        return out;
    }

    void forward(const __half* sample, double timestep, const __half* ehs_in, int ehs_rows, const float* added_ids, __half* out) {
        void* splitk = nullptr;
        {
            const int down = 1 << (m.boc.size() - 1);
            const long long m_low = (long long)B * F * (h / down) * (w / down);
            if (tune_env("SYN3R_SPLITK", 1) != 0 && ((m_low + 255) / 256) * ((m.boc.back() + 159) / 160) * 2 <= 256) {
                const size_t bytes = (size_t)4 * m_low * m.boc.back() * 4;
                splitk = take(bytes);
                if (go()) chk(syn3r_gemm_set_splitk_workspace(splitk, bytes));
            }
        }
        forward_body(sample, timestep, ehs_in, ehs_rows, added_ids, out);
        if (splitk) {
            if (!dry) syn3r_gemm_set_splitk_workspace(nullptr, 0);
            ar.release(splitk);
        }
    }
    void forward_body(const __half* sample, double timestep, const __half* ehs_in, int ehs_rows, const float* added_ids, __half* out) {
        const int c0 = m.boc[0];
        T te = make(B, c0);
        launch1d(k_timestep_embedding, B * (c0 / 2), (const float*)nullptr, timestep, 0.0f, B, c0, te.p);
        T emb = embed_mlp("time_embedding", te);
        const int nid = m.proj_in / m.add_dim;
        T ta = make((long long)B * nid, m.add_dim);
        launch1d(k_timestep_embedding, B * nid * (m.add_dim / 2), added_ids, 0.0, 0.0f, B * nid, m.add_dim, ta.p);
        T ta2 = ta; ta2.rows = B; ta2.cols = nid * m.add_dim;
        T aug = embed_mlp("add_embedding", ta2);
        T es = make(emb.rows, emb.cols);
        launch1d(k_add, es.rows * es.cols, emb.p, aug.p, es.p, es.rows * es.cols);
        drop(emb);
        drop(aug);
        T act = silu(es);
        drop(es);
        temb_all = linear(act, "time_emb_proj.all.weight", "time_emb_proj.all.bias");
        drop(act);
        ehs.p = (__half*)ehs_in; ehs.rows = ehs_rows; ehs.cols = m.cross[0];
        const int CP = (m.in_ch + 63) / 64 * 64;
        T xin = make((long long)B * F * h * w, CP);
        launch1d(k_nchw_to_nhwc, xin.rows * CP, sample, xin.p, B * F, m.in_ch, h * w, CP);
        T x = conv3x3(xin, B * F, h, w, CP, "conv_in.weight", "conv_in.bias", 1, false, Epi());
        drop(xin);
        std::vector<T> skips{x};
        for (auto& bp : m.down) {
            const std::string bpre = "down_blocks." + std::to_string(bp.idx);
            for (size_t j = 0; j < bp.layers.size(); ++j) {
                T y = resblock(bpre + ".resnets." + std::to_string(j), x, bp.layers[j].first, bp.layers[j].second, nullptr);
                if (bp.attn) { T z = transformer(bpre + ".attentions." + std::to_string(j), y, bp.layers[j].second, bp.heads); drop(y); y = z; }
                x = y;
                skips.push_back(x);
            }
            if (bp.resample) {
                int Ho, Wo;
                T y = conv3x3(x, B * F, h, w, bp.ch, bpre + ".downsamplers.0.conv.weight", bpre + ".downsamplers.0.conv.bias", 2, false, Epi(), &Ho, &Wo);
                h = Ho; w = Wo;
                x = y;
                skips.push_back(x);
            }
        }
        {
            const int mid = m.boc.back();
            T y = resblock("mid_block.resnets.0", x, mid, mid, nullptr);
            T z = transformer("mid_block.attentions.0", y, mid, m.heads.back());
            drop(y);
            x = resblock("mid_block.resnets.1", z, mid, mid, nullptr);
            drop(z);
        }
        for (auto& bp : m.up) {
            const std::string bpre = "up_blocks." + std::to_string(bp.idx);
// ... 75 lines not shown
```

### syn3r_amd/tuning.py

```python
from __future__ import annotations

import os

FLAGS = {
    "ff_fused": True,
    "ff_ln": True,
    "ff_tiled": True,
    "ln_qkv": True,
    "splitk": True,
    "unet_cat": False,
    "unet_graph": False,
    "two_streams": True,
    "merge_passes": True,
    "ff_g256": True,
    "gn_epilogue": True,
}

_ENV = {"ff_fused": "SYN3R_FF_FUSED", "ff_ln": "SYN3R_FF_LN", "ff_tiled": "SYN3R_FF_TILED", "ln_qkv": "SYN3R_LN_QKV",
        "splitk": "SYN3R_SPLITK", "unet_cat": "SYN3R_UNET_CAT", "unet_graph": "SYN3R_UNET_GRAPH",
        "two_streams": "SYN3R_TWO_STREAMS", "merge_passes": "SYN3R_MERGE_PASSES", "gn_epilogue": "SYN3R_GN_EPILOGUE", "ff_g256": "SYN3R_FF_G256"}


def from_env() -> dict:
    for key, name in _ENV.items():
        v = os.environ.get(name)
        if v is not None:
            FLAGS[key] = v != "0"
    return FLAGS
```

### syn3r_amd/unet/model.py

```python
from __future__ import annotations

import math
from typing import Dict, Optional, Sequence, Tuple, Union

import torch
import torch.nn.functional as Fn

from .. import _lib as L
from ..tuning import FLAGS as TUNE
from . import ops

H = torch.float16


def timestep_embedding(t: torch.Tensor, dim: int) -> torch.Tensor:
    half = dim // 2
    exponent = -math.log(10000) * torch.arange(half, dtype=torch.float32, device=t.device) / half
    emb = t[:, None].float() * torch.exp(exponent)[None, :]
    return torch.cat([torch.cos(emb), torch.sin(emb)], dim=-1)


class _Params:

    def __init__(self):
# ... 300 lines not shown
        hcur = ops.groupnorm(x, W(s + ".norm1.weight"), W(s + ".norm1.bias"), B * F, 1e-5, True, x2=x2)
        hcur = ops.conv3x3(hcur.view(B * F, h, w_, cin), W(s + ".conv1.weight"), W(s + ".conv1.bias"),
                           rowvec=tp_s, rows_per_vec=F * HW, gn_stats=TUNE["gn_epilogue"])
        hcur = ops.keep_gn(hcur.view(-1, cout), hcur)
        hcur = ops.groupnorm(hcur, W(s + ".norm2.weight"), W(s + ".norm2.bias"), B * F, 1e-5, True)
        skip = x
        if x2 is not None:
            skip = ops.linear_cat(x, x2, W(s + ".conv_shortcut.weight"), W(s + ".conv_shortcut.bias"))
        elif cin != cout:
            skip = ops.linear(x, W(s + ".conv_shortcut.weight"), W(s + ".conv_shortcut.bias"))
        xs = ops.conv3x3(hcur.view(B * F, h, w_, cout), W(s + ".conv2.weight"), W(s + ".conv2.bias"),
                         residual=skip, gn_stats=TUNE["gn_epilogue"])
        xs = ops.keep_gn(xs.view(-1, cout), xs)
        a0, a1 = self._temb_slices[t + ".time_emb_proj"]
        tp_t = st["temb_all"][:, a0:a1]
        hcur = ops.groupnorm(xs, W(t + ".norm1.weight"), W(t + ".norm1.bias"), B, 1e-5, True)
        hcur = ops.tconv3(hcur, W(t + ".conv1.weight"), W(t + ".conv1.bias"), B, F, HW, rowvec=tp_t, rows_per_vec=F * HW, gn_stats=TUNE["gn_epilogue"])
        hcur = ops.groupnorm(hcur, W(t + ".norm2.weight"), W(t + ".norm2.bias"), B, 1e-5, True)
        a, om = self._blend_scales(pre + ".time_mixer.mix_factor")
        return ops.tconv3(hcur, W(t + ".conv2.weight"), W(t + ".conv2.bias"), B, F, HW, residual=xs, s_acc=om,
                          s_res=a + om, gn_stats=TUNE["gn_epilogue"])

    def _cross_vec(self, pre: str, ehs: torch.Tensor, cache: Optional[dict] = None) -> torch.Tensor:
        if cache is not None and pre in cache:
            return cache[pre]
        v = ops.linear(ehs, self.w(pre + ".to_v.weight"))
        out = ops.linear(v, self.w(pre + ".to_out.0.weight"), self.w(pre + ".to_out.0.bias"))
        if cache is not None:
            cache[pre] = out
        return out

    def _ff(self, pre: str, x: torch.Tensor, norm: Optional[str] = None, addvec: Optional[tuple] = None, **epilogue) -> torch.Tensor:
        D = self.p.shapes[pre + ".net.0.proj.weight"][0] // 2
        cw = self.packed.get(pre + ".net.0.proj.geglu_cw")
        fuse = TUNE["ff_ln"]
        if addvec is not None and not (cw is not None and fuse):
            x, hmix = ops.layernorm(x, self.w(norm + ".weight"), self.w(norm + ".bias"), addvec=addvec[0], rows_per_vec=addvec[1],
                                    want_sum=True)
            norm, addvec, epilogue = None, None, dict(epilogue, residual=hmix)
        if cw is not None:
            ln = (self.w(norm + ".weight"), self.w(norm + ".bias"), 1e-5) if norm and fuse else None
            if norm and ln is None:
                x = ops.layernorm(x, self.w(norm + ".weight"), self.w(norm + ".bias"))
            return ops.feedforward_fused(x, cw, self.packed[pre + ".net.0.proj.geglu_cb"], D, self.w(pre + ".net.2.weight"),
                                         self.w(pre + ".net.2.bias"), ln=ln, addvec=addvec, **epilogue)
        if norm:
            x = ops.layernorm(x, self.w(norm + ".weight"), self.w(norm + ".bias"))
        wp = self.w(pre + ".net.0.proj.geglu_w")
        if not TUNE["ff_tiled"]:
            return ops.linear(ops.linear_geglu(x, wp, self.w(pre + ".net.0.proj.geglu_b"), D),
                              self.w(pre + ".net.2.weight"), self.w(pre + ".net.2.bias"), **epilogue)
        w64 = self.packed.get(pre + ".net.0.proj.geglu_w64") if TUNE["ff_g256"] else None
        p64 = (w64, self.packed[pre + ".net.0.proj.geglu_b64"]) if w64 is not None else None
        return ops.feedforward(x, wp, self.w(pre + ".net.0.proj.geglu_b"), D, self.w(pre + ".net.2.weight"),
                               self.w(pre + ".net.2.bias"), packed64=p64, **epilogue)

    def _norm_qkv(self, blk: str, x: torch.Tensor) -> torch.Tensor:
        W = self.w
        if not TUNE["ln_qkv"]:
            return ops.linear(ops.layernorm(x, W(blk + ".norm1.weight"), W(blk + ".norm1.bias")), W(blk + ".attn1.qkv"))
        return ops.layernorm_linear(x, W(blk + ".norm1.weight"), W(blk + ".norm1.bias"), W(blk + ".attn1.qkv"))

    def _transformer(self, pre: str, x: torch.Tensor, st: dict, ch: int, heads: int) -> torch.Tensor:
        B, F, h, w_ = st["B"], st["F"], st["h"], st["w"]
        HW = h * w_
        W = self.w
        ehs = st["ehs"]
        hs = ops.groupnorm(x, W(pre + ".norm.weight"), W(pre + ".norm.bias"), B * F, 1e-6, False)
        hs = ops.linear(hs, W(pre + ".proj_in.weight"), W(pre + ".proj_in.bias"))
        ck = (pre, F, B, str(x.device))
        emb = self._pos_cache.get(ck)
        if emb is None:
            pos = timestep_embedding(torch.arange(F, device=x.device), ch).to(H)
            e = ops.linear(pos, W(pre + ".time_pos_embed.linear_1.weight"), W(pre + ".time_pos_embed.linear_1.bias"))
            e = ops.linear(Fn.silu(e), W(pre + ".time_pos_embed.linear_2.weight"), W(pre + ".time_pos_embed.linear_2.bias"))
            emb = self._pos_cache[ck] = e.repeat(B, 1).contiguous()
        b = pre + ".transformer_blocks.0"
        a1 = ops.attention(self._norm_qkv(b, hs), B * F, HW, heads)
        hs = ops.linear(a1, W(b + ".attn1.to_out.0.weight"), W(b + ".attn1.to_out.0.bias"), residual=hs,
                        rowvec=self._cross_vec(b + ".attn2", ehs, st["ctx_cache"]), rows_per_vec=(B if st["shared_ctx"] else 1) * F * HW)
        hs = self._ff(b + ".ff", hs, norm=b + ".norm3", residual=hs)
        t = pre + ".temporal_transformer_blocks.0"
        tt = self._ff(t + ".ff_in", hs, norm=t + ".norm_in", addvec=(emb, HW))
        a1 = ops.attention_temporal(self._norm_qkv(t, tt), B, F, HW, heads)
        G = st["ctx_group"]
        if st["shared_ctx"]:
            rpv, grp = B * F * HW, 0
        elif G == 1:
            rpv, grp = F * HW, 0
        else:
            if HW % G:
                raise NotImplementedError("temporal cross-attention context interleave needs h*w divisible by the batch "
                                          "size (or one context shared by the batch: pass it expanded, stride 0)")
            rpv, grp = -G, (G * F * HW if G != B else 0)
        tt = ops.linear(a1, W(t + ".attn1.to_out.0.weight"), W(t + ".attn1.to_out.0.bias"), residual=tt,
                        rowvec=self._cross_vec(t + ".attn2", ehs, st["ctx_cache"]), rows_per_vec=rpv, rv_group_rows=grp)
        a, om = self._blend_scales(pre + ".time_mixer.mix_factor")
        mix = self._ff(t + ".ff", tt, norm=t + ".norm3", residual=tt, aux=hs, s_acc=om, s_res=om, s_aux=a)
        return ops.linear(mix, W(pre + ".proj_out.weight"), W(pre + ".proj_out.bias"), residual=x, gn_stats=TUNE["gn_epilogue"])

    @torch.no_grad()
    def forward(self, sample: torch.Tensor, timestep, encoder_hidden_states: torch.Tensor,
                added_time_ids: torch.Tensor, return_dict: bool = False, ctx_group: Optional[int] = None):
        if self.device is None:
            raise L.Syn3rError("UNet weights are not loaded (load_state_dict / from_pretrained / init_random)")
        dev = L.require_gpu(sample, encoder_hidden_states, added_time_ids)
        c = self.config
        B, F, Cin, h, w_ = sample.shape
        if Cin != c["in_channels"]:
            raise ValueError(f"sample has {Cin} channels, the model expects {c['in_channels']}")
        if F > 32:
            raise NotImplementedError("temporal attention kernel supports up to 32 frames")
        W = self.w
        boc = c["block_out_channels"]
        down = 2 ** (len(boc) - 1)
        m_low = B * F * (h // down) * (w_ // down)
        splitk = None
        if TUNE["splitk"] and ((m_low + 255) // 256) * ((boc[-1] + 159) // 160) * 2 <= 256:
            nbytes = 4 * m_low * boc[-1] * 4
            splitk = L.workspace(dev, nbytes, "splitk")
            L.check(L.load().syn3r_gemm_set_splitk_workspace(L.ptr(splitk), nbytes), "syn3r_gemm_set_splitk_workspace")
        try:
            return self._forward(sample, timestep, encoder_hidden_states, added_time_ids, return_dict, ctx_group)
        finally:
            if splitk is not None:
                L.load().syn3r_gemm_set_splitk_workspace(None, 0)

    def _forward(self, sample, timestep, encoder_hidden_states, added_time_ids, return_dict, ctx_group):
        dev = L.require_gpu(sample, encoder_hidden_states, added_time_ids)
        c = self.config
        B, F, Cin, h, w_ = sample.shape
        W = self.w
        boc = c["block_out_channels"]
        ts = timestep if torch.is_tensor(timestep) else torch.tensor([timestep], dtype=torch.float64)
        ts = ts.reshape(-1).to(dev).expand(B)
        t_emb = timestep_embedding(ts, boc[0]).to(H)
        emb = ops.linear(t_emb, W("time_embedding.linear_1.weight"), W("time_embedding.linear_1.bias"))
        emb = ops.linear(Fn.silu(emb), W("time_embedding.linear_2.weight"), W("time_embedding.linear_2.bias"))
        te = timestep_embedding(added_time_ids.flatten().to(dev), c["addition_time_embed_dim"]).reshape(B, -1).to(H)
        aug = ops.linear(te, W("add_embedding.linear_1.weight"), W("add_embedding.linear_1.bias"))
        aug = ops.linear(Fn.silu(aug), W("add_embedding.linear_2.weight"), W("add_embedding.linear_2.bias"))
        emb = emb + aug
        shared_ctx = B == 1 or encoder_hidden_states.stride(0) == 0
        ctx = encoder_hidden_states[:1] if shared_ctx else encoder_hidden_states
        G = B if ctx_group is None else int(ctx_group)
        if G < 1 or B % G:
            raise ValueError(f"ctx_group={ctx_group} must divide the batch size {B}")
        st = dict(B=B, F=F, h=h, w=w_, temb_act=Fn.silu(emb).contiguous(), shared_ctx=shared_ctx, ctx_group=G,
                  ehs=ctx.reshape(ctx.shape[0], -1).to(H).contiguous(), ctx_cache=self._context_cache(encoder_hidden_states, shared_ctx))
        st["temb_all"] = ops.linear(st["temb_act"], W("time_emb_proj.all.weight"), W("time_emb_proj.all.bias"))
        x = sample.to(H).flatten(0, 1).permute(0, 2, 3, 1)
        x = Fn.pad(x, (0, 64 - Cin % 64 if Cin % 64 else 0)).contiguous()
        x = ops.conv3x3(x, W("conv_in.weight"), W("conv_in.bias"), gn_stats=TUNE["gn_epilogue"])
        x = ops.keep_gn(x.view(-1, boc[0]), x)
        skips = [(x, boc[0])]
        for blk in self.down_plan:
            i = blk["idx"]
            for j, (cin, cout) in enumerate(blk["layers"]):
                x = self._resblock(f"down_blocks.{i}.resnets.{j}", x, st, cin, cout)
                if blk["attn"]:
                    x = self._transformer(f"down_blocks.{i}.attentions.{j}", x, st, cout, blk["heads"])
                skips.append((x, cout))
            if blk["down"]:
                ch = blk["ch"]
                x = ops.conv3x3(x.view(B * F, st["h"], st["w"], ch), W(f"down_blocks.{i}.downsamplers.0.conv.weight"),
                                W(f"down_blocks.{i}.downsamplers.0.conv.bias"), stride=2, gn_stats=TUNE["gn_epilogue"])
                st["h"], st["w"] = x.shape[1], x.shape[2]
                x = ops.keep_gn(x.view(-1, ch), x)
                skips.append((x, ch))
        mid = boc[-1]
        x = self._resblock("mid_block.resnets.0", x, st, mid, mid)
        x = self._transformer("mid_block.attentions.0", x, st, mid, c["num_attention_heads"][-1])
        x = self._resblock("mid_block.resnets.1", x, st, mid, mid)
        for blk in self.up_plan:
            i = blk["idx"]
            for j, (cin, cout) in enumerate(blk["layers"]):
                sk, sk_ch = skips.pop()
                if TUNE["unet_cat"]:
                    x = self._resblock(f"up_blocks.{i}.resnets.{j}", torch.cat([x, sk], dim=1), st, cin, cout)
# ... 56 lines not shown
```

### syn3r_amd/unet/ops.py

```python
from __future__ import annotations

import ctypes
from typing import Optional

import torch

from .. import _lib as L

H = torch.float16

FLOPS = {"enabled": False, "gemm": 0.0, "attn": 0.0}


def _count(kind: str, flops: float) -> None:
    if FLOPS["enabled"]:
        FLOPS[kind] += flops


def _chk(*ts):
    dev = L.require_gpu(*[t for t in ts if t is not None])
    for t in ts:
        if t is not None and (t.dtype != H or not t.is_contiguous()):
            raise L.Syn3rError(f"UNet operators need contiguous fp16 tensors, got {t.dtype} contiguous={t.is_contiguous()}")
    return dev
# ... 202 lines not shown
def pack_upsample4(weight: torch.Tensor) -> torch.Tensor:
    if weight.dim() != 4 or tuple(weight.shape[1:3]) != (3, 3):
        raise ValueError(f"pack_upsample4: weight {tuple(weight.shape)} is not [Cout,3,3,Cin]")
    groups = (((0,), (1, 2)), ((0, 1), (2,)))
    w = weight.float()
    out = torch.empty((4, weight.shape[0], 2, 2, weight.shape[3]), dtype=H, device=weight.device)
    for py in range(2):
        for px in range(2):
            for a in range(2):
                for b in range(2):
                    acc = None
                    for ty in groups[py][a]:
                        for tx in groups[px][b]:
                            acc = w[:, ty, tx] if acc is None else acc + w[:, ty, tx]
                    out[2 * py + px, :, a, b] = acc.to(H)
    return out


def conv3x3_up4(x: torch.Tensor, w4: torch.Tensor, bias: Optional[torch.Tensor] = None, *, gn_stats: bool = False) -> torch.Tensor:
    dev = _chk(x, w4, bias)
    NB, Hi, Wi, Cin = x.shape
    if w4.dim() != 5 or w4.shape[0] != 4 or tuple(w4.shape[2:]) != (2, 2, Cin):
        raise ValueError(f"conv3x3_up4: w4 {tuple(w4.shape)} does not match Cin={Cin}")
    Cout = w4.shape[1]
    out = torch.empty((NB, 2 * Hi, 2 * Wi, Cout), dtype=H, device=dev)
    lib = L.load()
    part, gn = _gn_request(dev, NB * 4 * Hi * Wi, Cout, gn_stats)
    rc = lib.syn3r_conv2d3x3_up4_f16(L.ptr(x), L.ptr(w4), L.ptr(out), L.ptr(bias), None, NB, Hi, Wi, Cin, Cout, *gn, L.stream_ptr(dev))
    L.check(rc, "syn3r_conv2d3x3_up4_f16")
    _count("gemm", 2.0 * NB * 4 * Hi * Wi * Cout * 4 * Cin)
    return _gn_collect(out, part, gn[2])


def tconv3(x: torch.Tensor, weight: torch.Tensor, bias: Optional[torch.Tensor], B: int, F: int, HW: int, *,
           rowvec: Optional[torch.Tensor] = None, rows_per_vec: int = 0, residual: Optional[torch.Tensor] = None,
           s_acc: float = 1.0, s_res: float = 1.0, gn_stats: bool = False) -> torch.Tensor:
    dev = _chk(x, weight, bias, residual)
    rv_ptr, rv_ld = _rowvec(rowvec)
    M, Cin = x.shape
    Cout = weight.shape[0]
    if M != B * F * HW or tuple(weight.shape[1:]) != (3, Cin):
        raise ValueError("tconv3: shape mismatch")
    out = torch.empty((M, Cout), dtype=H, device=dev)
    lib = L.load()
    part, gn = _gn_request(dev, M, Cout, gn_stats)
    rc = lib.syn3r_tconv3_f16(L.ptr(x), L.ptr(weight), L.ptr(out), Cout, L.ptr(bias), rv_ptr, rv_ld, int(rows_per_vec), L.ptr(residual),
                              Cout if residual is not None else 0, float(s_acc), float(s_res), B, F, HW, Cin, Cout, *gn,
                              L.stream_ptr(dev))
    L.check(rc, "syn3r_tconv3_f16")
    _count("gemm", 2.0 * M * Cout * 3 * Cin)
    return _gn_collect(out, part, gn[2])


def attention(qkv: torch.Tensor, nseq: int, S: int, heads: int) -> torch.Tensor:
    dev = _chk(qkv)
    C = heads * 64
    if qkv.shape != (nseq * S, 3 * C):
        raise ValueError(f"attention: qkv {tuple(qkv.shape)} != {(nseq * S, 3 * C)}")
    out = torch.empty((nseq * S, C), dtype=H, device=dev)
    base = qkv.data_ptr()
    lib = L.load()
    rc = lib.syn3r_attention_f16(base, base + 2 * C, base + 4 * C, 3 * C, L.ptr(out), C, nseq, S, heads,
                                 L.stream_ptr(dev))
    L.check(rc, "syn3r_attention_f16")
    _count("attn", 4.0 * nseq * heads * S * S * 64)
    return out


def attention_temporal(qkv: torch.Tensor, B: int, F: int, HW: int, heads: int) -> torch.Tensor:
    dev = _chk(qkv)
    C = heads * 64
    if qkv.shape != (B * F * HW, 3 * C):
        raise ValueError(f"attention_temporal: qkv {tuple(qkv.shape)} != {(B * F * HW, 3 * C)}")
    out = torch.empty((B * F * HW, C), dtype=H, device=dev)
    base = qkv.data_ptr()
    lib = L.load()
    rc = lib.syn3r_attention_temporal_f16(base, base + 2 * C, base + 4 * C, 3 * C, L.ptr(out), C, B, F, HW, heads,
                                          L.stream_ptr(dev))
    L.check(rc, "syn3r_attention_temporal_f16")
    _count("attn", 4.0 * B * HW * heads * F * F * 64)
    return out


def groupnorm(x: torch.Tensor, gamma: torch.Tensor, beta: torch.Tensor, samples: int, eps: float, silu: bool,
              x2: Optional[torch.Tensor] = None, use_partials: bool = True) -> torch.Tensor:
    dev = _chk(x, gamma, beta, x2)
    M, C = x.shape
    if M % samples:
        raise ValueError("groupnorm: rows not divisible by samples")
    lib = L.load()
    ws = L.workspace(dev, lib.syn3r_groupnorm_workspace_bytes(samples, M // samples), "gn")
    p1 = getattr(x, "gn_part", None) if use_partials else None
    p2 = getattr(x2, "gn_part", None) if (use_partials and x2 is not None) else None
    Ct = C + (x2.shape[1] if x2 is not None else 0)
    if p1 is not None and (x2 is None or p2 is not None) and (M // samples) % 32 == 0 and Ct % 320 == 0 and C % 10 == 0:
        if x2 is not None and x2.shape[0] != M:
            raise ValueError("groupnorm: the two sources must have the same rows")
        y = torch.empty((M, Ct), dtype=H, device=dev)
        rc = lib.syn3r_groupnorm_pre_f16(L.ptr(x), C, L.ptr(p1), L.ptr(x2), Ct - C, L.ptr(p2), L.ptr(y), samples, M // samples,
                                         L.ptr(gamma), L.ptr(beta), float(eps), 1 if silu else 0, L.ptr(ws), ws.numel(), L.stream_ptr(dev))
        L.check(rc, "syn3r_groupnorm_pre_f16")
        return y
    if x2 is not None:
        if x2.shape[0] != M:
            raise ValueError("groupnorm: the two sources must have the same rows")
        C2 = x2.shape[1]
        y = torch.empty((M, C + C2), dtype=H, device=dev)
        rc = lib.syn3r_groupnorm_2src_f16(L.ptr(x), C, L.ptr(x2), C2, L.ptr(y), samples, M // samples, L.ptr(gamma), L.ptr(beta),
                                          float(eps), 1 if silu else 0, L.ptr(ws), ws.numel(), L.stream_ptr(dev))
        L.check(rc, "syn3r_groupnorm_2src_f16")
        return y
    y = torch.empty_like(x)
    rc = lib.syn3r_groupnorm_f16(L.ptr(x), L.ptr(y), samples, M // samples, C, L.ptr(gamma), L.ptr(beta), float(eps),
                                 1 if silu else 0, L.ptr(ws), ws.numel(), L.stream_ptr(dev))
    L.check(rc, "syn3r_groupnorm_f16")
    return y


def linear_cat(x1: torch.Tensor, x2: torch.Tensor, weight: torch.Tensor, bias: Optional[torch.Tensor] = None) -> torch.Tensor:
    dev = L.require_gpu(x1, x2, weight)
    M, K1 = x1.shape
    K2 = x2.shape[1]
    N = weight.shape[0]
    if x2.shape[0] != M or weight.shape[1] != K1 + K2 or x1.stride(1) != 1 or x2.stride(1) != 1:
        raise ValueError(f"linear_cat: x1 {tuple(x1.shape)} / x2 {tuple(x2.shape)} / weight {tuple(weight.shape)} mismatch")
    _chk(weight, bias)
    lib = L.load()
    if not lib.syn3r_gemm_2src_supported(M, N, K1, K2, x1.stride(0), x2.stride(0)):
        return linear(torch.cat([x1, x2], dim=1), weight, bias)
    out = torch.empty((M, N), dtype=H, device=dev)
    rc = lib.syn3r_gemm_2src_f16(x1.data_ptr(), x1.stride(0), K1, x2.data_ptr(), x2.stride(0), K2, L.ptr(weight), out.data_ptr(),
                                 out.stride(0), L.ptr(bias), M, N, None, 0, None, L.stream_ptr(dev))
    L.check(rc, "syn3r_gemm_2src_f16")
    _count("gemm", 2.0 * M * N * (K1 + K2))
    return out


def layernorm_linear(x: torch.Tensor, gamma: torch.Tensor, beta: torch.Tensor, weight: torch.Tensor, eps: float = 1e-5) -> torch.Tensor:
    dev = _chk(gamma, beta, weight)
    L.require_gpu(x)
    M, K = x.shape
    N = weight.shape[0]
    if weight.shape[1] != K or gamma.numel() != K or beta.numel() != K or x.stride(1) != 1:
        raise ValueError(f"layernorm_linear: x {tuple(x.shape)} / weight {tuple(weight.shape)} / norm {gamma.numel()} mismatch")
    if K != FUSED_FF_CHANNELS or N % FUSED_FF_CHANNELS or x.stride(0) % 8 or x.data_ptr() % 16:
        return linear(layernorm(x.contiguous(), gamma, beta, eps), weight)
    out = torch.empty((M, N), dtype=H, device=dev)
    rc = L.load().syn3r_layernorm_linear320_f16(x.data_ptr(), x.stride(0), L.ptr(gamma), L.ptr(beta), float(eps), L.ptr(weight),
                                                out.data_ptr(), out.stride(0), M, N, K, L.stream_ptr(dev))
    L.check(rc, "syn3r_layernorm_linear320_f16")
    _count("gemm", 2.0 * M * N * K)
    return out


def layernorm(x: torch.Tensor, gamma: torch.Tensor, beta: torch.Tensor, eps: float = 1e-5, *,
              addvec: Optional[torch.Tensor] = None, rows_per_vec: int = 0, want_sum: bool = False):
    dev = _chk(x, gamma, beta, addvec)
    M, C = x.shape
    y = torch.empty_like(x)
    xsum = torch.empty_like(x) if (want_sum and addvec is not None) else None
    lib = L.load()
    rc = lib.syn3r_layernorm_f16(L.ptr(x), L.ptr(y), L.ptr(xsum), L.ptr(addvec), int(rows_per_vec), M, C,
                                 L.ptr(gamma), L.ptr(beta), float(eps), L.stream_ptr(dev))
    L.check(rc, "syn3r_layernorm_f16")
    return (y, xsum) if want_sum else y

# ... 38 lines not shown
```

Before: 419.1 iters/s.

## Fuse LayerNorm, QKV GEMM, temporal attention and out-projection into one kernel

Adds a single kernel for the C=320 temporal transformer attention block. It applies LayerNorm, runs the QKV projection into LDS, does per-pixel temporal attention from LDS, then applies the output projection with bias, rowvec and residual epilogue. This replaces three launches and drops the global round-trips of the qkv and attention-output intermediates. The attention core is factored into a shared header so the standalone kernel and the fused one use the same code. The fused path is on by default behind an env/tune flag and only covers C=320 layers where HW divides the pixels-per-block. The UNet is a small part of a loop dominated by 50 raster iterations, so the end-to-end effect is diluted.

```diff
diff --git a/include/syn3r_hip.h b/include/syn3r_hip.h
--- a/include/syn3r_hip.h
+++ b/include/syn3r_hip.h
@@ -220,6 +220,12 @@
 int syn3r_layernorm_linear320_f16(const void* x, long long ldx, const void* ln_gamma, const void* ln_beta, float ln_eps,
                                   const void* W, void* out, long long ldc, int M, int N, int C, void* stream);
 
+int syn3r_temporal_attention_block320_supported(int B, int F, int HW, int C);
+int syn3r_temporal_attention_block320_f16(const void* x, long long ldx, const void* ln_gamma, const void* ln_beta, float ln_eps,
+                                          const void* wqkv, const void* wout, const void* bout, const void* rowvec, long long ldrv,
+                                          int rows_per_vec, int rv_group_rows, void* out, long long ldc, int B, int F, int HW, int C,
+                                          void* stream);
+
 int syn3r_conv2d3x3_f16(const void* X, const void* W, void* out, long long ldc, const void* bias,
                         const void* rowvec, long long ldrv, int rows_per_vec, const void* residual, long long ldr,
                         float s_acc, float s_res, int NB, int Hi, int Wi, int Cin, int Cout, int stride, int upsample,
diff --git a/syn3r_amd/_lib.py b/syn3r_amd/_lib.py
--- a/syn3r_amd/_lib.py
+++ b/syn3r_amd/_lib.py
@@ -92,6 +92,9 @@
     "syn3r_feedforward_fused_addln_f16": (c_i, [c_p, c_ll, c_p, c_i, c_p, c_p, c_f, c_p, c_p, c_i, c_p, c_p, c_p, c_ll, c_p, c_ll,
                                                 c_f, c_f, c_f, c_i, c_i, c_p]),
     "syn3r_layernorm_linear320_f16": (c_i, [c_p, c_ll, c_p, c_p, c_f, c_p, c_p, c_ll, c_i, c_i, c_i, c_p]),
+    "syn3r_temporal_attention_block320_supported": (c_i, [c_i, c_i, c_i, c_i]),
+    "syn3r_temporal_attention_block320_f16": (c_i, [c_p, c_ll, c_p, c_p, c_f, c_p, c_p, c_p, c_p, c_ll, c_i, c_i, c_p, c_ll, c_i, c_i, c_i,
+                                                   c_i, c_p]),
     "syn3r_conv2d3x3_f16": (c_i, [c_p, c_p, c_p, c_ll, c_p, c_p, c_ll, c_i, c_p, c_ll, c_f, c_f,
                                   c_i, c_i, c_i, c_i, c_i, c_i, c_i, c_i, c_p, c_sz, C.POINTER(c_i), c_p]),
     "syn3r_pack_upsample4_f16": (c_i, [c_p, c_p, c_i, c_i]),
diff --git a/syn3r_amd/csrc/attn.hip b/syn3r_amd/csrc/attn.hip
--- a/syn3r_amd/csrc/attn.hip
+++ b/syn3r_amd/csrc/attn.hip
@@ -11,31 +11,12 @@
 typedef float float2v __attribute__((ext_vector_type(2)));
 typedef __fp16 fp16x4 __attribute__((__vector_size__(4 * sizeof(__fp16))));
 
-__device__ __forceinline__ int v_off(int key, int d) { return key * 64 + ((((d >> 3) ^ (((key >> 1) & 1) << 2)) << 3) | (d & 7)); }
+#include "attn_temporal_core.h"
+
 __device__ __forceinline__ int k_off(int key, int chunk) { return key * 64 + ((chunk ^ ((key >> 1) & 7)) << 3); }
 
-__device__ __forceinline__ half8 v_frag_tr(const __half* vs, int r0, int d0, int lane) {
-    const int i = lane & 15, q = i >> 2, pc = i & 3;
-    const int c = d0 + ((lane >> 4) & 1) * 16 + 4 * pc;
-    typedef __attribute__((address_space(3))) fp16x4 lds4;
-    fp16x4 a = __builtin_amdgcn_ds_read_tr16_b64_v4f16((lds4*)(vs + v_off(r0 + q, c)));
-    fp16x4 b = __builtin_amdgcn_ds_read_tr16_b64_v4f16((lds4*)(vs + v_off(r0 + 8 + q, c)));
-    half8 r;
-#pragma unroll
-    for (int e = 0; e < 4; ++e) { r[e] = (_Float16)a[e]; r[4 + e] = (_Float16)b[e]; }
-    return r;
-}
-
-constexpr float kNegBig = -1.0e30f;
 constexpr float kLog2e = 1.4426950408889634f;
 constexpr float kLazy = 8.0f;
-
-__device__ __forceinline__ half8 pack8(const float16v& p, int s) {
-    half8 r;
-#pragma unroll
-    for (int j = 0; j < 8; ++j) r[j] = (_Float16)p[8 * s + j];
-    return r;
-}
 
 struct AttnParams {
     const __half* q; const __half* k; const __half* v;
@@ -274,6 +255,24 @@
     }
 }
 
+struct TemporalGlobalSrc {
+    const __half* qb; const __half* kb; const __half* vb;
+    long long fstride;
+    __device__ __forceinline__ half8 q(int f, int c) const { return *(const half8*)(qb + f * fstride + c * 8); }
+    __device__ __forceinline__ half8 k(int f, int c) const { return *(const half8*)(kb + f * fstride + c * 8); }
+    __device__ __forceinline__ void stage_v(__half* vs, int F, int lane) const {
+#pragma unroll
+        for (int i = 0; i < 4; ++i) {
+            int q = lane + 64 * i;
+            int key = q >> 3, ch = q & 7;
+            uint4 rv = make_uint4(0, 0, 0, 0);
+            if (key < F) rv = *(const uint4*)(vb + key * fstride + ch * 8);
+            *(uint4*)(vs + v_off(key, ch * 8)) = rv;
+        }
+    }
+    __device__ __forceinline__ void v_ready() const { __syncthreads(); }
+};
+
 __global__ void __launch_bounds__(ATHREADS, 2) k_attn_temporal(AttnParams p, long long nitems) {
     __shared__ __attribute__((aligned(16))) __half Vsm[4][32 * 64];
     const int tid = threadIdx.x, lane = tid & 63, wv = tid >> 6;
@@ -288,74 +287,16 @@
     const int F = p.F;
     auto row_of = [&](int f) { return ((long long)b * F + f) * p.HW + pix; };
 
-    const int fq = lq < F ? lq : F - 1;
-    const __half* qsrc = p.q + row_of(fq) * p.ld + hd * 64;
-    const __half* ksrc = p.k + row_of(fq) * p.ld + hd * 64;
-    half8 qf[4], kf[4];
-#pragma unroll
-    for (int ks = 0; ks < 4; ++ks) {
-        half8 t = *(const half8*)(qsrc + ks * 16 + 8 * h);
-#pragma unroll
-        for (int j = 0; j < 8; ++j) t[j] = t[j] * (_Float16)0.125f;
-        qf[ks] = t;
-        kf[ks] = *(const half8*)(ksrc + ks * 16 + 8 * h);
-    }
-    __half* vs = Vsm[wv];
-#pragma unroll
-    for (int i = 0; i < 4; ++i) {
-        int q = lane + 64 * i;
-        int key = q >> 3, ch = q & 7;
-        uint4 rv = make_uint4(0, 0, 0, 0);
-        if (key < F) rv = *(const uint4*)(p.v + row_of(key) * p.ld + hd * 64 + ch * 8);
-        *(uint4*)(vs + v_off(key, ch * 8)) = rv;
-    }
-    float16v st;
-#pragma unroll
-    for (int r = 0; r < 16; ++r) st[r] = 0.f;
-#pragma unroll
-    for (int ks = 0; ks < 4; ++ks) st = __builtin_amdgcn_mfma_f32_32x32x16_f16(kf[ks], qf[ks], st, 0, 0, 0);
-    float mx = kNegBig;
-#pragma unroll
-    for (int r = 0; r < 16; ++r) {
-        int key = (r & 3) + 8 * (r >> 2) + 4 * h;
-        if (key >= F) st[r] = kNegBig;
-        mx = fmaxf(mx, st[r]);
-    }
-    mx = fmaxf(mx, __shfl_xor(mx, 32, 64));
-    float ls = 0.f;
-#pragma unroll
-    for (int r = 0; r < 16; ++r) {
-        float e = __expf(st[r] - mx);
-        st[r] = e;
-        ls += e;
-    }
-    ls += __shfl_xor(ls, 32, 64);
-    __syncthreads();
-    float16v ot[2];
-#pragma unroll
-    for (int r = 0; r < 16; ++r) { ot[0][r] = 0.f; ot[1][r] = 0.f; }
-#pragma unroll
-    for (int s = 0; s < 2; ++s) {
-        half8 pf = pack8(st, s);
-#pragma unroll
-        for (int dt = 0; dt < 2; ++dt) {
-            half8 vf = v_frag_tr(vs, s * 16 + 4 * h, dt * 32, lane);
-            ot[dt] = __builtin_amdgcn_mfma_f32_32x32x16_f16(vf, pf, ot[dt], 0, 0, 0);
-        }
-    }
-    if (live && lq < F) {
-        const float inv = 1.0f / ls;
-        __half* dst = p.o + row_of(lq) * p.ldo + hd * 64;
-#pragma unroll
-        for (int dt = 0; dt < 2; ++dt)
-#pragma unroll
-            for (int g = 0; g < 4; ++g) {
-                half4 o4;
-#pragma unroll
-                for (int e = 0; e < 4; ++e) o4[e] = (_Float16)(ot[dt][4 * g + e] * inv);
-                *(half4*)(dst + dt * 32 + 8 * g + 4 * h) = o4;
-            }
-    }
+    TemporalGlobalSrc src;
+    src.qb = p.q + row_of(0) * p.ld + hd * 64;
+    src.kb = p.k + row_of(0) * p.ld + hd * 64;
+    src.vb = p.v + row_of(0) * p.ld + hd * 64;
+    src.fstride = (long long)p.HW * p.ld;
+    const bool store = live && lq < F;
+    __half* dst = p.o + row_of(lq < F ? lq : F - 1) * p.ldo + hd * 64;
+    attn_temporal_core(src, Vsm[wv], F, lane, [&](int dt, int g, half4 o4) {
+        if (store) *(half4*)(dst + dt * 32 + 8 * g + 4 * h) = o4;
+    });
 }
 
 }
diff --git a/syn3r_amd/csrc/attn_temporal_core.h b/syn3r_amd/csrc/attn_temporal_core.h
--- /dev/null
+++ b/syn3r_amd/csrc/attn_temporal_core.h
@@ -0,0 +1,82 @@
+typedef _Float16 half8 __attribute__((ext_vector_type(8)));
+typedef _Float16 half4 __attribute__((ext_vector_type(4)));
+typedef float float16v __attribute__((ext_vector_type(16)));
+typedef __fp16 fp16x4 __attribute__((__vector_size__(4 * sizeof(__fp16))));
+
+__device__ __forceinline__ int v_off(int key, int d) { return key * 64 + ((((d >> 3) ^ (((key >> 1) & 1) << 2)) << 3) | (d & 7)); }
+
+__device__ __forceinline__ half8 v_frag_tr(const __half* vs, int r0, int d0, int lane) {
+    const int i = lane & 15, q = i >> 2, pc = i & 3;
+    const int c = d0 + ((lane >> 4) & 1) * 16 + 4 * pc;
+    typedef __attribute__((address_space(3))) fp16x4 lds4;
+    fp16x4 a = __builtin_amdgcn_ds_read_tr16_b64_v4f16((lds4*)(vs + v_off(r0 + q, c)));
+    fp16x4 b = __builtin_amdgcn_ds_read_tr16_b64_v4f16((lds4*)(vs + v_off(r0 + 8 + q, c)));
+    half8 r;
+#pragma unroll
+    for (int e = 0; e < 4; ++e) { r[e] = (_Float16)a[e]; r[4 + e] = (_Float16)b[e]; }
+    return r;
+}
+
+constexpr float kNegBig = -1.0e30f;
+
+__device__ __forceinline__ half8 pack8(const float16v& p, int s) {
+    half8 r;
+#pragma unroll
+    for (int j = 0; j < 8; ++j) r[j] = (_Float16)p[8 * s + j];
+    return r;
+}
+
+template <class Src, class Out>
+__device__ __forceinline__ void attn_temporal_core(const Src& src, __half* vs, int F, int lane, const Out& out) {
+    const int lq = lane & 31, h = lane >> 5;
+    const int fq = lq < F ? lq : F - 1;
+    half8 qf[4], kf[4];
+#pragma unroll
+    for (int ks = 0; ks < 4; ++ks) {
+        half8 t = src.q(fq, ks * 2 + h);
+#pragma unroll
+        for (int j = 0; j < 8; ++j) t[j] = t[j] * (_Float16)0.125f;
+        qf[ks] = t;
+        kf[ks] = src.k(fq, ks * 2 + h);
+    }
+    src.stage_v(vs, F, lane);
+    float16v st;
+#pragma unroll
+    for (int r = 0; r < 16; ++r) st[r] = 0.f;
+#pragma unroll
+    for (int ks = 0; ks < 4; ++ks) st = __builtin_amdgcn_mfma_f32_32x32x16_f16(kf[ks], qf[ks], st, 0, 0, 0);
+    float mx = kNegBig;
+#pragma unroll
+    for (int r = 0; r < 16; ++r) {
+        int key = (r & 3) + 8 * (r >> 2) + 4 * h;
+        if (key >= F) st[r] = kNegBig;
+        mx = fmaxf(mx, st[r]);
+    }
+    mx = fmaxf(mx, __shfl_xor(mx, 32, 64));
+    float ls = 0.f;
+#pragma unroll
+    for (int r = 0; r < 16; ++r) {
+        float e = __expf(st[r] - mx);
+        st[r] = e;
+        ls += e;
+    }
+    ls += __shfl_xor(ls, 32, 64);
+    const float inv = 1.0f / ls;
+    const half8 pf[2] = {pack8(st, 0), pack8(st, 1)};
+    src.v_ready();
+#pragma unroll
+    for (int dt = 0; dt < 2; ++dt) {
+        float16v ot;
+#pragma unroll
+        for (int r = 0; r < 16; ++r) ot[r] = 0.f;
+#pragma unroll
+        for (int s = 0; s < 2; ++s) ot = __builtin_amdgcn_mfma_f32_32x32x16_f16(v_frag_tr(vs, s * 16 + 4 * h, dt * 32, lane), pf[s], ot, 0, 0, 0);
+#pragma unroll
+        for (int g = 0; g < 4; ++g) {
+            half4 o4;
+#pragma unroll
+            for (int e = 0; e < 4; ++e) o4[e] = (_Float16)(ot[4 * g + e] * inv);
+            out(dt, g, o4);
+        }
+    }
+}
diff --git a/syn3r_amd/csrc/gemm.hip b/syn3r_amd/csrc/gemm.hip
--- a/syn3r_amd/csrc/gemm.hip
+++ b/syn3r_amd/csrc/gemm.hip
@@ -17,6 +17,8 @@
 #include "gemm_dmapd.h"
 #include "gemm_g256.h"
 #include "gemm_ffn.h"
+#include "attn_temporal_core.h"
+#include "gemm_tattn.h"
 
 int persistent_blocks() {
     static std::atomic<int> cus_of[64];
@@ -530,6 +532,34 @@
     return launch_lnlin320(p, (hipStream_t)stream);
 }
 
+extern "C" int syn3r_temporal_attention_block320_supported(int B, int F, int HW, int C) {
+    return (C == F_C && SYN3R_DIM_OK(B) && SYN3R_DIM_OK(HW) && F >= 1 && F <= 32 && (long long)B * F * HW <= SYN3R_DIM_MAX &&
+            HW % tattn_pixels_per_block(F) == 0) ? 1 : 0;
+}
+
+extern "C" int syn3r_temporal_attention_block320_f16(const void* x, long long ldx, const void* ln_gamma, const void* ln_beta, float ln_eps,
+                                                     const void* wqkv, const void* wout, const void* bout, const void* rowvec, long long ldrv,
+                                                     int rows_per_vec, int rv_group_rows, void* out, long long ldc, int B, int F, int HW, int C,
+                                                     void* stream) {
+    SYN3R_REQUIRE(x && ln_gamma && ln_beta && wqkv && wout && out, "temporal_attention_block320_f16: null operand");
+    SYN3R_REQUIRE(C == F_C, "temporal_attention_block320_f16: the kernel is built for C = %d channels (got %d): use the three launches", F_C, C);
+    SYN3R_REQUIRE(SYN3R_DIM_OK(B) && SYN3R_DIM_OK(HW) && F >= 1 && F <= 32 && (long long)B * F * HW <= SYN3R_DIM_MAX,
+                  "temporal_attention_block320_f16: bad sizes B=%d F=%d HW=%d (F <= 32)", B, F, HW);
+    SYN3R_REQUIRE(ldx % 8 == 0 && ldx >= C && ldc % 8 == 0 && ldc >= C, "temporal_attention_block320_f16: bad strides ldx=%lld ldc=%lld", ldx, ldc);
+    SYN3R_REQUIRE(((uintptr_t)x | (uintptr_t)ln_gamma | (uintptr_t)ln_beta | (uintptr_t)wqkv | (uintptr_t)wout | (uintptr_t)bout | (uintptr_t)out) % 16 == 0,
+                  "temporal_attention_block320_f16: operands must be 16-byte aligned");
+    SYN3R_REQUIRE(x != out, "temporal_attention_block320_f16: out must not alias x (a block reads rows other blocks write)");
+    SYN3R_REQUIRE(ln_eps > 0.f, "temporal_attention_block320_f16: eps must be positive");
+    SYN3R_REQUIRE(!rowvec || (rows_per_vec != 0 && ldrv >= C && ldrv % 4 == 0 && (uintptr_t)rowvec % 8 == 0), "temporal_attention_block320_f16: bad rowvec arguments");
+    SYN3R_REQUIRE(rv_group_rows >= 0 && (rv_group_rows == 0 || rows_per_vec < 0), "temporal_attention_block320_f16: rv_group_rows needs rows_per_vec < 0");
+    TattnParams p{};
+    p.x = (const __half*)x; p.ldx = ldx; p.wqkv = (const __half*)wqkv; p.wout = (const __half*)wout; p.bias = (const __half*)bout;
+    p.rowvec = (const __half*)rowvec; p.ldrv = ldrv; p.rows_per_vec = rows_per_vec; p.rv_group = rv_group_rows;
+    p.out = (__half*)out; p.ldc = ldc; p.ln_g = (const __half*)ln_gamma; p.ln_b = (const __half*)ln_beta; p.ln_eps = ln_eps;
+    p.B = B; p.F = F; p.HW = HW; p.C = C;
+    return launch_tattn320(p, (hipStream_t)stream);
+}
+
 extern "C" int syn3r_conv2d3x3_f16(const void* X, const void* W, void* out, long long ldc, const void* bias,
                                    const void* rowvec, long long ldrv, int rows_per_vec, const void* residual,
                                    long long ldr, float s_acc, float s_res, int NB, int Hi, int Wi, int Cin, int Cout,
diff --git a/syn3r_amd/csrc/gemm_tattn.h b/syn3r_amd/csrc/gemm_tattn.h
--- /dev/null
+++ b/syn3r_amd/csrc/gemm_tattn.h
@@ -0,0 +1,424 @@
+constexpr int T_Q = 0, T_K = 16384, T_V = 32768, T_RING = 65536, T_SLOT = 16384;
+constexpr int T_LDS = T_RING + 6 * T_SLOT;
+
+struct TattnParams {
+    const __half* x; long long ldx;
+    const __half* wqkv;
+    const __half* wout;
+    const __half* bias;
+    const __half* rowvec; long long ldrv; int rows_per_vec, rv_group;
+    __half* out; long long ldc;
+    const __half* ln_g; const __half* ln_b; float ln_eps;
+    int B, F, HW, C;
+};
+
+struct TemporalLdsSrc {
+    const char* qt; const char* kt;
+    int row0;
+    __device__ __forceinline__ half8 q(int f, int c) const { const int r = row0 + f; return *(const half8*)(qt + r * 128 + ((c ^ (r & 7)) << 4)); }
+    __device__ __forceinline__ half8 k(int f, int c) const { const int r = row0 + f; return *(const half8*)(kt + r * 128 + ((c ^ (r & 7)) << 4)); }
+    __device__ __forceinline__ void stage_v(__half*, int, int) const {}
+    __device__ __forceinline__ void v_ready() const {}
+};
+
+template <bool G32>
+__global__ void __launch_bounds__(512, 2) k_tattn320(TattnParams p) {
+    constexpr int RPP = G32 ? 32 : 16, PPB = F_BM / RPP;
+    extern __shared__ __attribute__((aligned(16))) char smem_raw[];
+    const int tid = threadIdx.x, lane = tid & 63;
+    const int wv = __builtin_amdgcn_readfirstlane(tid >> 6);
+    const int wm = wv >> 1, wn = wv & 1;
+    const int fr = lane & 15, fq = lane >> 4;
+    const int F = p.F;
+    const int npix = p.B * p.HW;
+    const int pix0 = (int)xcd_remap(blockIdx.x, gridDim.x) * PPB;
+    typedef _Float16 half4e __attribute__((ext_vector_type(4)));
+    auto row_of = [&](int r, bool& real) -> int {
+        const int f = r % RPP;
+        int gp = pix0 + r / RPP;
+        real = gp < npix && f < F;
+        gp = gp < npix ? gp : npix - 1;
+        const int b = gp / p.HW, pix = gp - b * p.HW;
+        return (b * F + (f < F ? f : F - 1)) * p.HW + pix;
+    };
+
+    half8 xf[2][10];
+#pragma unroll
+    for (int i = 0; i < 2; ++i) {
+        bool real;
+        const int m = row_of(wm * 32 + i * 16 + fr, real);
+        const __half* xr = p.x + (long long)m * p.ldx + fq * 8;
+#pragma unroll
+        for (int ks = 0; ks < 10; ++ks) xf[i][ks] = *(const half8*)(xr + ks * 32);
+    }
+
+    const int prow = lane >> 3;
+    const int csrc = (lane & 7) ^ prow;
+    unsigned o_lane = (unsigned)((prow * F_C + csrc * 8) * 2);
+    const int r_qk = (wv >> 2) * 320 + (wv & 3) * 16;
+    const int r_v = 640 + wv * 8;
+    const int r_u = (wv >> 2) * 160 + (wv & 3) * 16;
+    const int r_u2 = (wv >> 2) * 160 + 128 + (wv & 3) * 8;
+    char* const ring = smem_raw + T_RING;
+    auto dma = [&](const __half* base, long long soff, unsigned& lane_off, char* dst) {
+        asm volatile("" : "+s"(soff), "+v"(lane_off));
+        __builtin_amdgcn_global_load_lds((gbl_void_t*)((const char*)base + soff + (size_t)lane_off), (lds_void_t*)dst, 16, 0, 0);
+    };
+    auto issue = [&](auto ST, int h) {
+        constexpr int st = decltype(ST)::value;
+        if constexpr (st < 5) {
+#pragma unroll
+            for (int i = 0; i < 2; ++i)
+                dma(p.wqkv, ((long long)(r_qk + h * 64 + i * 8) * F_C + st * 64) * 2, o_lane, ring + st * T_SLOT + (wv * 2 + i) * 1024);
+        } else if constexpr (st < 8) {
+            constexpr int slot = st == 5 ? 5 : st - 6, kt0 = (st - 5) * 2, nk = st == 7 ? 1 : 2;
+#pragma unroll
+            for (int kk = 0; kk < nk; ++kk)
+                dma(p.wqkv, ((long long)(r_v + h * 64) * F_C + (kt0 + kk) * 64) * 2, o_lane, ring + slot * T_SLOT + kk * 8192 + wv * 1024);
+        } else if constexpr (st == 9 || st == 10) {
+            constexpr int slot = st - 7, jt0 = (st - 9) * 4;
+#pragma unroll
+            for (int i = 0; i < 2; ++i)
+                dma(p.wout, ((long long)(r_u + jt0 * 16 + i * 8) * F_C + h * 64) * 2, o_lane, ring + slot * T_SLOT + (wv * 2 + i) * 1024);
+        } else if constexpr (st == 11) {
+            dma(p.wout, ((long long)r_u2 * F_C + h * 64) * 2, o_lane, ring + 4 * T_SLOT + wv * 1024);
+        }
+    };
+    issue(std::integral_constant<int, 0>{}, 0);
+    issue(std::integral_constant<int, 1>{}, 0);
+    issue(std::integral_constant<int, 2>{}, 0);
+    issue(std::integral_constant<int, 3>{}, 0);
+    __builtin_amdgcn_sched_barrier(0);
+#pragma unroll
+    for (int i = 0; i < 2; ++i)
+#pragma unroll
+        for (int ks = 0; ks < 10; ++ks) asm volatile("" : "+v"(xf[i][ks]));
+
+    {
+        const float cf = (float)p.C;
+        float mean[2], rstd[2];
+#pragma unroll
+        for (int i = 0; i < 2; ++i) {
+            float sa = 0.f, sb = 0.f;
+#pragma unroll
+            for (int k = 0; k < 5; ++k)
+#pragma unroll
+                for (int e = 0; e < 8; ++e) { sa += (float)xf[i][2 * k][e]; sb += (float)xf[i][2 * k + 1][e]; }
+            float s = sa + sb;
+            s += __shfl_xor(s, 32, 64);
+            s += __shfl_xor(s, 16, 64);
+            mean[i] = s / cf;
+            float qa = 0.f, qb = 0.f;
+            {
+#pragma clang fp contract(off)
+#pragma unroll
+                for (int k = 0; k < 5; ++k)
+#pragma unroll
+                    for (int e = 0; e < 8; ++e) {
+                        const float da = (float)xf[i][2 * k][e] - mean[i], db = (float)xf[i][2 * k + 1][e] - mean[i];
+                        const float da2 = da * da, db2 = db * db;
+                        qa += da2; qb += db2;
+                    }
+            }
+            float qq = qa + qb;
+            qq += __shfl_xor(qq, 32, 64);
+            qq += __shfl_xor(qq, 16, 64);
+            rstd[i] = rsqrtf(qq / cf + p.ln_eps);
+        }
+#pragma unroll
+        for (int k5 = 0; k5 < 10; k5 += 5) {
+            half8 g[5], b[5];
+#pragma unroll
+            for (int ks = 0; ks < 5; ++ks) { g[ks] = *(const half8*)(p.ln_g + (k5 + ks) * 32 + fq * 8); b[ks] = *(const half8*)(p.ln_b + (k5 + ks) * 32 + fq * 8); }
+            __builtin_amdgcn_sched_barrier(0);
+#pragma unroll
+            for (int ks = 0; ks < 5; ++ks) asm volatile("" : "+v"(g[ks]), "+v"(b[ks]));
+#pragma unroll
+            for (int ks = 0; ks < 5; ++ks)
+#pragma unroll
+                for (int i = 0; i < 2; ++i) {
+                    half8 o;
+#pragma unroll
+                    for (int e = 0; e < 8; ++e) o[e] = (_Float16)(((float)xf[i][k5 + ks][e] - mean[i]) * rstd[i] * (float)g[ks][e] + (float)b[ks][e]);
+                    xf[i][k5 + ks] = o;
+                }
+        }
+    }
+    {
+        uint4* vz = (uint4*)(smem_raw + T_V);
+#pragma unroll
+        for (int i = 0; i < 4; ++i) vz[tid + i * 512] = make_uint4(0, 0, 0, 0);
+    }
+    __syncthreads();
+
+    float4v acc[2][10];
+#pragma unroll
+    for (int i = 0; i < 2; ++i)
+#pragma unroll
+        for (int j = 0; j < 10; ++j) acc[i][j] = (float4v){0.f, 0.f, 0.f, 0.f};
+
+    const unsigned lds0 = lds_addr(smem_raw);
+    const unsigned la0 = lds0 + (unsigned)(fr * 128 + (((0 + fq) ^ (fr & 7)) << 4)), la1 = lds0 + (unsigned)(fr * 128 + (((4 + fq) ^ (fr & 7)) << 4));
+    auto fresh = [](unsigned v) { asm volatile("" : "+v"(v)); return v; };
+    const unsigned u_w64 = (unsigned)(T_RING + wn * 64 * 128), u_w32 = (unsigned)(T_RING + wn * 32 * 128), u_a = (unsigned)(T_Q + wm * 32 * 128);
+
+#define T_BAR() do { asm volatile("s_waitcnt lgkmcnt(0)" ::: "memory"); __builtin_amdgcn_s_barrier(); } while (0)
+#define T_MF4(B, KS, SS)                                                                                                  \
+    _Pragma("unroll") for (int i = 0; i < 2; ++i)                                                                         \
+        _Pragma("unroll") for (int t = 0; t < 4; ++t) SS[i][t] = __builtin_amdgcn_mfma_f32_16x16x32_f16(B[t], xf[i][KS], SS[i][t], 0, 0, 0); \
+    __builtin_amdgcn_sched_barrier(0);
+
+    for (int h = 0; h < 5; ++h) {
+        const bool more = h + 1 < 5;
+        float4v S[2][4];
+#pragma unroll
+        for (int i = 0; i < 2; ++i)
+#pragma unroll
+            for (int t = 0; t < 4; ++t) S[i][t] = (float4v){0.f, 0.f, 0.f, 0.f};
+        auto step_qk = [&](auto KT, auto NEXT) {
+            constexpr int kt = decltype(KT)::value;
+            if constexpr (kt < 4) asm volatile("s_waitcnt vmcnt(6)" ::: "memory");
+            else asm volatile("s_waitcnt vmcnt(5)" ::: "memory");
+            T_BAR();
+            const unsigned wa0 = fresh(la0) + (u_w64 + (unsigned)(kt * T_SLOT)), wa1 = fresh(la1) + (u_w64 + (unsigned)(kt * T_SLOT));
+            half8 b0[4], b1[4];
+            DS_READ128(b0[0], wa0, 0); DS_READ128(b0[1], wa0, 2048); DS_READ128(b0[2], wa0, 4096); DS_READ128(b0[3], wa0, 6144);
+            DS_READ128(b1[0], wa1, 0); DS_READ128(b1[1], wa1, 2048); DS_READ128(b1[2], wa1, 4096); DS_READ128(b1[3], wa1, 6144);
+            issue(NEXT, h);
+            asm volatile("s_waitcnt lgkmcnt(4)" : "+v"(b0[0]), "+v"(b0[1]), "+v"(b0[2]), "+v"(b0[3]));
+            T_MF4(b0, 2 * kt, S)
+            asm volatile("s_waitcnt lgkmcnt(0)" : "+v"(b1[0]), "+v"(b1[1]), "+v"(b1[2]), "+v"(b1[3]));
+            T_MF4(b1, 2 * kt + 1, S)
+        };
+        step_qk(std::integral_constant<int, 0>{}, std::integral_constant<int, 4>{});
+        step_qk(std::integral_constant<int, 1>{}, std::integral_constant<int, 5>{});
+        step_qk(std::integral_constant<int, 2>{}, std::integral_constant<int, 6>{});
+        step_qk(std::integral_constant<int, 3>{}, std::integral_constant<int, 7>{});
+        step_qk(std::integral_constant<int, 4>{}, std::integral_constant<int, 9>{});
+        const unsigned qk_z = fresh((unsigned)(((fq >> 1) ^ (fr & 7)) << 4));
+        const unsigned qk_wr = fresh(lds0 + (unsigned)(fr * 128 + (fq & 1) * 8)) + (unsigned)((wn ? T_K : T_Q) + wm * 32 * 128);
+#pragma unroll
+        for (int i = 0; i < 2; ++i)
+#pragma unroll
+            for (int t = 0; t < 4; ++t) {
+                half4e o;
+#pragma unroll
+                for (int r = 0; r < 4; ++r) o[r] = (_Float16)S[i][t][r];
+                DS_WRITE64(qk_wr + (unsigned)(i * 2048) + ((unsigned)(t * 32) ^ qk_z), o);
+            }
+
+#pragma unroll
+        for (int i = 0; i < 2; ++i)
+#pragma unroll
+            for (int t = 0; t < 2; ++t) S[i][t] = (float4v){0.f, 0.f, 0.f, 0.f};
+#define T_MF2(B0, B1, KS)                                                                                                 \
+    _Pragma("unroll") for (int i = 0; i < 2; ++i) {                                                                       \
+        S[i][0] = __builtin_amdgcn_mfma_f32_16x16x32_f16(B0, xf[i][KS], S[i][0], 0, 0, 0);                                \
+        S[i][1] = __builtin_amdgcn_mfma_f32_16x16x32_f16(B1, xf[i][KS], S[i][1], 0, 0, 0);                                \
+    }                                                                                                                     \
+    __builtin_amdgcn_sched_barrier(0);
+        auto step_v2 = [&](auto KT0, auto SLOT, auto NEXT) {
+            constexpr int kt0 = decltype(KT0)::value, slot = decltype(SLOT)::value;
+            asm volatile("s_waitcnt vmcnt(5)" ::: "memory");
+            T_BAR();
+            const unsigned wa0 = fresh(la0) + (u_w32 + (unsigned)(slot * T_SLOT)), wa1 = fresh(la1) + (u_w32 + (unsigned)(slot * T_SLOT));
+            half8 b[8];
+            DS_READ128(b[0], wa0, 0); DS_READ128(b[1], wa0, 2048); DS_READ128(b[2], wa1, 0); DS_READ128(b[3], wa1, 2048);
+            DS_READ128(b[4], wa0, 8192); DS_READ128(b[5], wa0, 10240); DS_READ128(b[6], wa1, 8192); DS_READ128(b[7], wa1, 10240);
+            issue(NEXT, h);
+            asm volatile("s_waitcnt lgkmcnt(4)" : "+v"(b[0]), "+v"(b[1]), "+v"(b[2]), "+v"(b[3]));
+            T_MF2(b[0], b[1], 2 * kt0)
+            T_MF2(b[2], b[3], 2 * kt0 + 1)
+            asm volatile("s_waitcnt lgkmcnt(0)" : "+v"(b[4]), "+v"(b[5]), "+v"(b[6]), "+v"(b[7]));
+            T_MF2(b[4], b[5], 2 * kt0 + 2)
+            T_MF2(b[6], b[7], 2 * kt0 + 3)
+        };
+        step_v2(std::integral_constant<int, 0>{}, std::integral_constant<int, 5>{}, std::integral_constant<int, 10>{});
+        step_v2(std::integral_constant<int, 2>{}, std::integral_constant<int, 0>{}, std::integral_constant<int, 11>{});
+        {
+            asm volatile("s_waitcnt vmcnt(5)" ::: "memory");
+            T_BAR();
+            const unsigned wa0 = fresh(la0) + (u_w32 + (unsigned)(1 * T_SLOT)), wa1 = fresh(la1) + (u_w32 + (unsigned)(1 * T_SLOT));
+            half8 b[4];
+            DS_READ128(b[0], wa0, 0); DS_READ128(b[1], wa0, 2048); DS_READ128(b[2], wa1, 0); DS_READ128(b[3], wa1, 2048);
+            asm volatile("s_waitcnt lgkmcnt(0)" : "+v"(b[0]), "+v"(b[1]), "+v"(b[2]), "+v"(b[3]));
+            T_MF2(b[0], b[1], 8)
+            T_MF2(b[2], b[3], 9)
+        }
+#undef T_MF2
+        const int fq4 = (int)fresh((unsigned)(fq * 4));
+#pragma unroll
+        for (int i = 0; i < 2; ++i) {
+            const int pl = G32 ? wm : wm * 2 + i, f = G32 ? i * 16 + fr : fr;
+#pragma unroll
+            for (int t = 0; t < 2; ++t) {
+                half4e o;
+#pragma unroll
+                for (int r = 0; r < 4; ++r) o[r] = f < F ? (_Float16)S[i][t][r] : (_Float16)0.f;
+                DS_WRITE64(lds0 + T_V + (unsigned)(pl * 4096 + v_off(f, wn * 32 + t * 16 + fq4) * 2), o);
+            }
+        }
+
+        asm volatile("s_waitcnt lgkmcnt(0)" ::: "memory");
+        __syncthreads();
+        if (wv < PPB) {
+            TemporalLdsSrc src;
+            src.qt = smem_raw + T_Q; src.kt = smem_raw + T_K; src.row0 = wv * RPP;
+            const int lq = lane & 31, hh = lane >> 5;
+            const int r = wv * RPP + (lq & (RPP - 1));
+            char* const arow = smem_raw + T_Q + r * 128 + hh * 8;
+            attn_temporal_core(src, (__half*)(smem_raw + T_V + wv * 4096), F, lane, [&](int dt, int g, half4 o4) {
+                if (lq < RPP) *(half4*)(arow + (((dt * 4 + g) ^ (r & 7)) << 4)) = o4;
+            });
+        }
+
+        if (more) { issue(std::integral_constant<int, 0>{}, h + 1); issue(std::integral_constant<int, 1>{}, h + 1); }
+
+        auto step_out4 = [&](auto JT0, auto SLOT, auto NEXT) {
+            constexpr int jt0 = decltype(JT0)::value, slot = decltype(SLOT)::value;
+            if constexpr (jt0 == 0) { if (more) asm volatile("s_waitcnt vmcnt(7)" ::: "memory"); else asm volatile("s_waitcnt vmcnt(3)" ::: "memory"); }
+            else { if (more) asm volatile("s_waitcnt vmcnt(5)" ::: "memory"); else asm volatile("s_waitcnt vmcnt(1)" ::: "memory"); }
+            T_BAR();
+            const unsigned f0 = fresh(la0), f1 = fresh(la1);
+            const unsigned wa0 = f0 + (u_w64 + (unsigned)(slot * T_SLOT)), wa1 = f1 + (u_w64 + (unsigned)(slot * T_SLOT)), aa0 = f0 + u_a, aa1 = f1 + u_a;
+            half8 af[2][2], b0[4], b1[4];
+            DS_READ128(af[0][0], aa0, 0); DS_READ128(af[1][0], aa0, 2048);
+            DS_READ128(b0[0], wa0, 0); DS_READ128(b0[1], wa0, 2048); DS_READ128(b0[2], wa0, 4096); DS_READ128(b0[3], wa0, 6144);
+            DS_READ128(af[0][1], aa1, 0); DS_READ128(af[1][1], aa1, 2048);
+            DS_READ128(b1[0], wa1, 0); DS_READ128(b1[1], wa1, 2048); DS_READ128(b1[2], wa1, 4096); DS_READ128(b1[3], wa1, 6144);
+            if (more) issue(NEXT, h + 1);
+            asm volatile("s_waitcnt lgkmcnt(6)" : "+v"(af[0][0]), "+v"(af[1][0]), "+v"(b0[0]), "+v"(b0[1]), "+v"(b0[2]), "+v"(b0[3]));
+#pragma unroll
+            for (int i = 0; i < 2; ++i)
+#pragma unroll
+                for (int t = 0; t < 4; ++t) acc[i][jt0 + t] = __builtin_amdgcn_mfma_f32_16x16x32_f16(b0[t], af[i][0], acc[i][jt0 + t], 0, 0, 0);
+            __builtin_amdgcn_sched_barrier(0);
+            asm volatile("s_waitcnt lgkmcnt(0)" : "+v"(af[0][1]), "+v"(af[1][1]), "+v"(b1[0]), "+v"(b1[1]), "+v"(b1[2]), "+v"(b1[3]));
+#pragma unroll
+            for (int i = 0; i < 2; ++i)
+#pragma unroll
+                for (int t = 0; t < 4; ++t) acc[i][jt0 + t] = __builtin_amdgcn_mfma_f32_16x16x32_f16(b1[t], af[i][1], acc[i][jt0 + t], 0, 0, 0);
+            __builtin_amdgcn_sched_barrier(0);
+        };
+        step_out4(std::integral_constant<int, 0>{}, std::integral_constant<int, 2>{}, std::integral_constant<int, 8>{});
+        step_out4(std::integral_constant<int, 4>{}, std::integral_constant<int, 3>{}, std::integral_constant<int, 2>{});
+        {
+            if (more) asm volatile("s_waitcnt vmcnt(6)" ::: "memory");
+            else asm volatile("s_waitcnt vmcnt(0)" ::: "memory");
+            T_BAR();
+            const unsigned f0 = fresh(la0), f1 = fresh(la1);
+            const unsigned wa0 = f0 + (u_w32 + (unsigned)(4 * T_SLOT)), wa1 = f1 + (u_w32 + (unsigned)(4 * T_SLOT)), aa0 = f0 + u_a, aa1 = f1 + u_a;
+            half8 af[2][2], b[4];
+            DS_READ128(af[0][0], aa0, 0); DS_READ128(af[1][0], aa0, 2048); DS_READ128(af[0][1], aa1, 0); DS_READ128(af[1][1], aa1, 2048);
+            DS_READ128(b[0], wa0, 0); DS_READ128(b[1], wa0, 2048); DS_READ128(b[2], wa1, 0); DS_READ128(b[3], wa1, 2048);
+            if (more) issue(std::integral_constant<int, 3>{}, h + 1);
+            asm volatile("s_waitcnt lgkmcnt(0)" : "+v"(af[0][0]), "+v"(af[1][0]), "+v"(af[0][1]), "+v"(af[1][1]), "+v"(b[0]), "+v"(b[1]), "+v"(b[2]), "+v"(b[3]));
+#pragma unroll
+            for (int kk = 0; kk < 2; ++kk)
+#pragma unroll
+                for (int i = 0; i < 2; ++i)
+#pragma unroll
+                    for (int t = 0; t < 2; ++t) acc[i][8 + t] = __builtin_amdgcn_mfma_f32_16x16x32_f16(b[kk * 2 + t], af[i][kk], acc[i][8 + t], 0, 0, 0);
+            __builtin_amdgcn_sched_barrier(0);
+        }
+    }
+#undef T_MF4
+#undef T_BAR
+    asm volatile("s_waitcnt vmcnt(0)" ::: "memory");
+    __syncthreads();
+
+    {
+        const int gn0 = wn * 160;
+        const int le = (int)fresh((unsigned)lane), fr = le & 15, fq = le >> 4;
+        __half* st = (__half*)smem_raw + wv * (32 * 168);
+        half8 res[10];
+        int mrow[10];
+#pragma unroll
+        for (int it = 0; it < 10; ++it) {
+            const int qi = le + it * 64;
+            const int row = qi / 20, ch = qi - row * 20;
+            bool real;
+            const int m = row_of(wm * 32 + row, real);
+            res[it] = *(const half8*)(p.x + (long long)m * p.ldx + gn0 + ch * 8);
+            mrow[it] = real ? m : -1;
+        }
+        const __half* rv[2];
+#pragma unroll
+        for (int i = 0; i < 2; ++i) {
+            bool real;
+            const int m = row_of(wm * 32 + i * 16 + fr, real);
+            rv[i] = p.rowvec ? p.rowvec + (long long)rowvec_index(m, p.rows_per_vec, p.rv_group) * p.ldrv : nullptr;
+        }
+        half4e bq[10], rq[2][10];
+        const half4e z4 = (half4e){(_Float16)0.f, (_Float16)0.f, (_Float16)0.f, (_Float16)0.f};
+        if (p.bias) {
+#pragma unroll
+            for (int jt = 0; jt < 10; ++jt) bq[jt] = *(const half4e*)(p.bias + gn0 + jt * 16 + fq * 4);
+        } else {
+#pragma unroll
+            for (int jt = 0; jt < 10; ++jt) bq[jt] = z4;
+        }
+        if (p.rowvec) {
+#pragma unroll
+            for (int i = 0; i < 2; ++i)
+#pragma unroll
+                for (int jt = 0; jt < 10; ++jt) rq[i][jt] = *(const half4e*)(rv[i] + gn0 + jt * 16 + fq * 4);
+        } else {
+#pragma unroll
+            for (int i = 0; i < 2; ++i)
+#pragma unroll
+                for (int jt = 0; jt < 10; ++jt) rq[i][jt] = z4;
+        }
+#pragma unroll
+        for (int jt = 0; jt < 10; ++jt) {
+            float b4[4];
+#pragma unroll
+            for (int r = 0; r < 4; ++r) b4[r] = (float)bq[jt][r];
+#pragma unroll
+            for (int i = 0; i < 2; ++i) {
+                float a4[4] = {b4[0], b4[1], b4[2], b4[3]};
+                if (p.rowvec) {
+#pragma unroll
+                    for (int r = 0; r < 4; ++r) a4[r] += (float)rq[i][jt][r];
+                }
+                half4e o;
+#pragma unroll
+                for (int r = 0; r < 4; ++r) o[r] = (_Float16)(acc[i][jt][r] + a4[r]);
+                *(half4e*)(st + (i * 16 + fr) * 168 + jt * 16 + fq * 4) = o;
+            }
+        }
+        __builtin_amdgcn_wave_barrier();
+        __syncthreads();
+#pragma unroll
+        for (int it = 0; it < 10; ++it) {
+            const int qi = le + it * 64;
+            const int row = qi / 20, ch = qi - row * 20;
+            if (mrow[it] < 0) continue;
+            half8 v = *(const half8*)(st + row * 168 + ch * 8);
+#pragma unroll
+            for (int e = 0; e < 8; ++e) v[e] = (_Float16)((float)v[e] + (float)res[it][e]);
+            *(half8*)(p.out + (long long)mrow[it] * p.ldc + gn0 + ch * 8) = v;
+        }
+    }
+}
+
+inline int tattn_pixels_per_block(int F) { return F <= 16 ? 8 : 4; }
+
+int launch_tattn320(const TattnParams& p, hipStream_t stream) {
+    static DevOnce once16, once32;
+    const bool g32 = p.F > 16;
+    if (int rc = g32 ? set_max_lds(once32, (const void*)k_tattn320<true>, T_LDS, "hipFuncSetAttribute(tattn320<32>)")
+                     : set_max_lds(once16, (const void*)k_tattn320<false>, T_LDS, "hipFuncSetAttribute(tattn320<16>)")) return rc;
+    const int ppb = tattn_pixels_per_block(p.F);
+    const long long npix = (long long)p.B * p.HW;
+    const int blocks = (int)((npix + ppb - 1) / ppb);
+    char name[96];
+    if (trace_on()) {
+        if (trace_detail()) snprintf(name, sizeof(name), "k_gemm_tattn320[M%lld,F%d]", npix * p.F, p.F);
+        else snprintf(name, sizeof(name), "k_gemm_tattn320");
+    }
+    if (g32) SYN3R_LAUNCH_NAMED(name, k_tattn320<true>, dim3(blocks), dim3(512), T_LDS, stream, p);
+    else SYN3R_LAUNCH_NAMED(name, k_tattn320<false>, dim3(blocks), dim3(512), T_LDS, stream, p);
+    SYN3R_LAUNCH_CHECK("tattn320 launch");
+    return SYN3R_OK;
+}
diff --git a/syn3r_amd/csrc/unet.hip b/syn3r_amd/csrc/unet.hip
--- a/syn3r_amd/csrc/unet.hip
+++ b/syn3r_amd/csrc/unet.hip
@@ -73,7 +73,7 @@
     std::unordered_map<std::string, Wt> w;
     struct PosEmb { __half* p = nullptr; hipEvent_t ready = nullptr; hipStream_t stream = nullptr; };
     std::map<std::string, PosEmb> pos_cache;
-    bool ff_ln = true, ln_qkv = true;
+    bool ff_ln = true, ln_qkv = true, tattn_fused = true;
 };
 
 namespace {
@@ -106,6 +106,7 @@
     std::vector<HostPack>().swap(m->packs);
     m->ff_ln = tune_env("SYN3R_FF_LN", 1) != 0;
     m->ln_qkv = tune_env("SYN3R_LN_QKV", 1) != 0;
+    m->tattn_fused = tune_env("SYN3R_TATTN_FUSED", 1) != 0;
     *out = m.release();
     {
         std::lock_guard<std::mutex> lk(g_unet_mu);
@@ -521,9 +522,6 @@
             drop(hmix);
         }
         {
-            T qkv = norm_qkv(t, tt);
-            T a1 = attention_temporal(qkv, HW, heads);
-            drop(qkv);
             int rpv, grp;
             if (shared_ctx) { rpv = B * F * HW; grp = 0; }
             else if (G == 1) { rpv = F * HW; grp = 0; }
@@ -532,9 +530,22 @@
                 rpv = -G; grp = G != B ? G * F * HW : 0;
             }
             const T& cv = cross_vec(t + ".attn2");
-            Epi e; e.residual = &tt; e.rowvec = dry ? nullptr : cv.p; e.ldrv = cv.cols; e.rows_per_vec = rpv; e.rv_group = grp;
-            T o = linear(a1, t + ".attn1.to_out.0.weight", t + ".attn1.to_out.0.bias", e);
-            drop(a1);
+            const Wt* wq = W(t + ".attn1.qkv");
+            T o;
+            if (m.tattn_fused && m.ln_qkv && wq && wq->rows == 3 * tt.cols && syn3r_temporal_attention_block320_supported(B, F, HW, tt.cols)) {
+                o = make(tt.rows, tt.cols);
+                if (go())
+                    chk(syn3r_temporal_attention_block320_f16(tt.p, tt.cols, Wp(t + ".norm1.weight"), Wp(t + ".norm1.bias"), 1e-5f, wq->p,
+                                                              Wp(t + ".attn1.to_out.0.weight"), Wp(t + ".attn1.to_out.0.bias"), dry ? nullptr : cv.p, cv.cols,
+                                                              rpv, grp, o.p, o.cols, B, F, HW, tt.cols, stream));
+            } else {
+                T qkv = norm_qkv(t, tt);
+                T a1 = attention_temporal(qkv, HW, heads);
+                drop(qkv);
+                Epi e; e.residual = &tt; e.rowvec = dry ? nullptr : cv.p; e.ldrv = cv.cols; e.rows_per_vec = rpv; e.rv_group = grp;
+                o = linear(a1, t + ".attn1.to_out.0.weight", t + ".attn1.to_out.0.bias", e);
+                drop(a1);
+            }
             drop(tt);
             tt = o;
         }
diff --git a/syn3r_amd/tuning.py b/syn3r_amd/tuning.py
--- a/syn3r_amd/tuning.py
+++ b/syn3r_amd/tuning.py
@@ -7,6 +7,7 @@
     "ff_ln": True,
     "ff_tiled": True,
     "ln_qkv": True,
+    "tattn_fused": True,
     "splitk": True,
     "unet_cat": False,
     "unet_graph": False,
@@ -17,6 +18,7 @@
 }
 
 _ENV = {"ff_fused": "SYN3R_FF_FUSED", "ff_ln": "SYN3R_FF_LN", "ff_tiled": "SYN3R_FF_TILED", "ln_qkv": "SYN3R_LN_QKV",
+        "tattn_fused": "SYN3R_TATTN_FUSED",
         "splitk": "SYN3R_SPLITK", "unet_cat": "SYN3R_UNET_CAT", "unet_graph": "SYN3R_UNET_GRAPH",
         "two_streams": "SYN3R_TWO_STREAMS", "merge_passes": "SYN3R_MERGE_PASSES", "gn_epilogue": "SYN3R_GN_EPILOGUE", "ff_g256": "SYN3R_FF_G256"}
 
diff --git a/syn3r_amd/unet/model.py b/syn3r_amd/unet/model.py
--- a/syn3r_amd/unet/model.py
+++ b/syn3r_amd/unet/model.py
@@ -406,7 +406,6 @@
         hs = self._ff(b + ".ff", hs, norm=b + ".norm3", residual=hs)
         t = pre + ".temporal_transformer_blocks.0"
         tt = self._ff(t + ".ff_in", hs, norm=t + ".norm_in", addvec=(emb, HW))
-        a1 = ops.attention_temporal(self._norm_qkv(t, tt), B, F, HW, heads)
         G = st["ctx_group"]
         if st["shared_ctx"]:
             rpv, grp = B * F * HW, 0
@@ -417,8 +416,15 @@
                 raise NotImplementedError("temporal cross-attention context interleave needs h*w divisible by the batch "
                                           "size (or one context shared by the batch: pass it expanded, stride 0)")
             rpv, grp = -G, (G * F * HW if G != B else 0)
-        tt = ops.linear(a1, W(t + ".attn1.to_out.0.weight"), W(t + ".attn1.to_out.0.bias"), residual=tt,
-                        rowvec=self._cross_vec(t + ".attn2", ehs, st["ctx_cache"]), rows_per_vec=rpv, rv_group_rows=grp)
+        cv = self._cross_vec(t + ".attn2", ehs, st["ctx_cache"])
+        if TUNE["tattn_fused"] and TUNE["ln_qkv"] and ops.temporal_attention_block_supported(B, F, HW, ch):
+            tt = ops.temporal_attention_block(tt, W(t + ".norm1.weight"), W(t + ".norm1.bias"), W(t + ".attn1.qkv"),
+                                              W(t + ".attn1.to_out.0.weight"), W(t + ".attn1.to_out.0.bias"), B, F, HW,
+                                              rowvec=cv, rows_per_vec=rpv, rv_group_rows=grp)
+        else:
+            a1 = ops.attention_temporal(self._norm_qkv(t, tt), B, F, HW, heads)
+            tt = ops.linear(a1, W(t + ".attn1.to_out.0.weight"), W(t + ".attn1.to_out.0.bias"), residual=tt, rowvec=cv,
+                            rows_per_vec=rpv, rv_group_rows=grp)
         a, om = self._blend_scales(pre + ".time_mixer.mix_factor")
         mix = self._ff(t + ".ff", tt, norm=t + ".norm3", residual=tt, aux=hs, s_acc=om, s_res=om, s_aux=a)
         return ops.linear(mix, W(pre + ".proj_out.weight"), W(pre + ".proj_out.bias"), residual=x, gn_stats=TUNE["gn_epilogue"])
diff --git a/syn3r_amd/unet/ops.py b/syn3r_amd/unet/ops.py
--- a/syn3r_amd/unet/ops.py
+++ b/syn3r_amd/unet/ops.py
@@ -308,6 +308,28 @@
     return out
 
 
+def temporal_attention_block_supported(B: int, F: int, HW: int, C: int) -> bool:
+    return bool(L.load().syn3r_temporal_attention_block320_supported(int(B), int(F), int(HW), int(C)))
+
+
+def temporal_attention_block(x: torch.Tensor, gamma: torch.Tensor, beta: torch.Tensor, wqkv: torch.Tensor, wout: torch.Tensor,
+                             bout: Optional[torch.Tensor], B: int, F: int, HW: int, *, rowvec: Optional[torch.Tensor] = None,
+                             rows_per_vec: int = 0, rv_group_rows: int = 0, eps: float = 1e-5) -> torch.Tensor:
+    dev = _chk(x, gamma, beta, wqkv, wout, bout)
+    M, C = x.shape
+    if M != B * F * HW or tuple(wqkv.shape) != (3 * C, C) or tuple(wout.shape) != (C, C) or gamma.numel() != C or beta.numel() != C:
+        raise ValueError(f"temporal_attention_block: x {tuple(x.shape)} / wqkv {tuple(wqkv.shape)} / wout {tuple(wout.shape)} / B, F, HW = {B}, {F}, {HW} mismatch")
+    rv_ptr, rv_ld = _rowvec(rowvec)
+    out = torch.empty((M, C), dtype=H, device=dev)
+    rc = L.load().syn3r_temporal_attention_block320_f16(L.ptr(x), C, L.ptr(gamma), L.ptr(beta), float(eps), L.ptr(wqkv), L.ptr(wout), L.ptr(bout),
+                                                        rv_ptr, rv_ld, int(rows_per_vec), int(rv_group_rows), L.ptr(out), C, B, F, HW, C,
+                                                        L.stream_ptr(dev))
+    L.check(rc, "syn3r_temporal_attention_block320_f16")
+    _count("gemm", 2.0 * M * C * 4 * C)
+    _count("attn", 4.0 * B * HW * (C // 64) * F * F * 64)
+    return out
+
+
 def groupnorm(x: torch.Tensor, gamma: torch.Tensor, beta: torch.Tensor, samples: int, eps: float, silu: bool,
               x2: Optional[torch.Tensor] = None, use_partials: bool = True) -> torch.Tensor:
     dev = _chk(x, gamma, beta, x2)
```

Result: no change. 422.2 iters/s (median of 6 runs) (+0.7%).
